# zichunhao/lgn-autoencoder

Measured on AMD Instinct MI355X. Metric: jets/sec fwd+bwd, 30-particle maxdim=2 bs=512, higher is better.
Workload: dtype f64

## Files before the change

### include/lgn_amd.h

```cpp
#ifndef LGN_AMD_H
#define LGN_AMD_H

#include <stddef.h>
#include <stdint.h>

#ifdef __cplusplus
extern "C" {
#endif

#define LGN_AMD_ABI_VERSION 19

int lgn_abi_version(void);
const char* lgn_last_error(void);

int lgn_level_fwd_f64(int B, int N, int C, int CO, int decoder,
                      const double* s_in, const double* v_in, const double* p, const uint8_t* mask,
                      const double* ra, const double* rb, const double* rc,
                      const double* w0, const double* b0, const double* w1, const double* b1,
                      const double* wm0, const double* wm1,
                      double* ag0, double* ag1, double* s_out, double* v_out, void* stream);

int lgn_level_bwd_partial_rows(int B, int N, int decoder, int* rows_mix, int* rows_rad);
int lgn_level_rad_partial_len(int C, int decoder);
int lgn_level_jet_split(int B, int N);
// ... 51 lines not shown
  int n_rows, n_out, n_w;
  int n_terms, n_u, n_x;
  int n_units, static_kind;
  const int *row_ptr, *t_type, *t_a, *t_b;
  const double* t_coef;
  const int *out_dim, *out_nblk, *out_row0, *out_q0, *out_w0;
  const int *u_ptr, *u_row;
  const double* u_coef;
  const int *x_ptr, *x_row, *x_other;
  const double* x_coef;
  int h_out_w0[8];
} lgn_local_tables;

int lgn_local_fwd_f64(int nodes, int C, int CO, int Q, int Qout, const lgn_local_tables* t, const double* X, const double* U,
                      const double* wcat, double* out, void* stream);
int lgn_local_partial_rows(int nodes);
int lgn_local_bwd_f64(int nodes, int C, int CO, int Q, int Qout, const lgn_local_tables* t, const double* X, const double* U,
                      const double* wcat, const double* g_out, double* gU, double* gX, double* part, void* stream);

long long lgn_local_static_packed_doubles(int kind, int C, int CO);
int lgn_local_bwd_static_f64(int kind, int nodes, int C, int CO, const double* XT, const double* UT, const double* wcat,
                             const int* w0, double* wpacked, const double* goT, double* gUT, double* gXT, double* part,
                             double* gpacked, double* g_wcat, void* stream);
int lgn_local_fwd_static_f64(int kind, int nodes, int C, int CO, const double* XT, const double* UT, const double* wcat,
                             const int* w0, double* wpacked, double* outT, double* s_copy, int q_s, void* stream);

typedef struct lgn_net_desc {
  int B, N;
  int n_levels;
  int enc_channels[5];
  int dec_channels[5];
  int tau_s, tau_v;
  int mlp_hidden_mul;
  int mlp_nlin;
  int tau_v_in;
  const lgn_local_tables* enc_tables[4];
  const lgn_local_tables* dec_tables[4];
  int enc_Q[5], enc_qs[5], enc_qv[5];
  int dec_Q[5], dec_qs[5], dec_qv[5];
  int flags;
  int activation;
  int n_in_scalars;
  int latent_pool;
  int dec_N;
  int get_real;
  double jet_loss_scale;
} lgn_net_desc;
#define LGN_REAL_SUM 0
#define LGN_REAL_REAL 1
#define LGN_REAL_IMAG 2
#define LGN_REAL_MEAN 3
#define LGN_REAL_NORM 4
#define LGN_LOSS_CHAMFER 0
#define LGN_LOSS_MSE 1
#define LGN_LOSS_HUNGARIAN 2
typedef struct lgn_loss_desc {
  int kind;
  int abs_coord;
  int polar_coord;
  double scale;
} lgn_loss_desc;
#define LGN_POOL_MIN 0
#define LGN_POOL_MAX 1
#define LGN_POOL_MEAN 2
#define LGN_POOL_MIX 3
#define LGN_POOL(n, avg, o0, o1, o2, o3) ((n) | ((avg) << 3) | ((o0) << 4) | ((o1) << 6) | ((o2) << 8) | ((o3) << 10))
#define LGN_NET_NO_STATIC 1
#define LGN_NET_DEC_PAIRWISE 2
#define LGN_NET_LEVEL_V2 4
#define LGN_NET_MLP_V1 8
#define LGN_NET_MOMENTS_V1 16
#define LGN_NET_BWD_ORDERED 64
#define LGN_NET_DEC_UNFUSED 256
#define LGN_NET_MOMENTS_SPLIT 512
#define LGN_NET_MLP_BWD1 1024
#define LGN_NET_MLP_FULLTILE 2048
#define LGN_NET_LIVE_SCALARS 4096
#define LGN_NET_SPLIT_TAIL 128

#define LGN_LDS_LIMIT (160 * 1024)
long long lgn_encoder_end_lds_bytes(int N, int C0, int K, int CL, int Ts, int Tv, int pool);
long long lgn_decoder_end_lds_bytes(int N, int C0, int Tin, int CL);
long long lgn_junction_lds_bytes(int N, int CL, int Ts, int Tv, int pool, int C0);

int lgn_step_param_slots(const lgn_net_desc* d, int decoder);
long long lgn_step_workspace_doubles(const lgn_net_desc* d);
int lgn_step_fwd_bwd_f64(const lgn_net_desc* d, const double* params, double* grads, long long n_params,
                         const int64_t* enc_off, const int64_t* dec_off, const double* p4, const double* target,
                         const uint8_t* mask, const double* in_scalars, double* workspace, long long workspace_doubles,
                         double* recon, double* loss_part, const lgn_loss_desc* loss, int* assignment ,
                         int* status , void* stream);
#define LGN_FINALIZE_SCRATCH 2048
int lgn_step_finalize_f64(double* params, double* grads, long long n_params, const double* loss_part, int n_loss,
                          double l1_lambda, double* adam_m, double* adam_v, long long* step_dev,
                          double lr, double beta1, double beta2, double eps, int do_adam, double* loss_out, void* stream);
int lgn_step_train_f64(const lgn_net_desc* d, double* params, double* grads, long long n_params, const int64_t* enc_off,
                       const int64_t* dec_off, const double* p4, const double* target, const uint8_t* mask, const double* in_scalars,
                       double* workspace, long long workspace_doubles, double* recon, double* loss_part, int n_loss, double l1_lambda,
                       double* adam_m, double* adam_v, long long* step_dev, double lr, double beta1, double beta2, double eps,
                       int do_adam, double* loss_out, const lgn_loss_desc* loss, int* assignment ,
                       int* status , void* stream);

#define LGN_OPT_ADAM 0
#define LGN_OPT_RMSPROP 1
typedef struct {
  int kind;
  double l1_lambda, l2_lambda, lr, eps;
  double beta1, beta2;
  double alpha, momentum;
} lgn_optim_desc;
#define LGN_FINALIZE_OPT_SCRATCH 4096
int lgn_step_finalize_opt_f64(double* params, double* grads, long long n_params, const double* loss_part, int n_loss,
                              const lgn_optim_desc* opt, double* state_m, double* state_v, long long* step_dev, int do_step,
                              double* loss_out, void* stream);
int lgn_step_train_opt_f64(const lgn_net_desc* d, double* params, double* grads, long long n_params, const int64_t* enc_off,
                           const int64_t* dec_off, const double* p4, const double* target, const uint8_t* mask,
                           const double* in_scalars, double* workspace, long long workspace_doubles, double* recon,
                           double* loss_part, int n_loss, const lgn_optim_desc* opt, double* state_m, double* state_v,
                           long long* step_dev, int do_step, double* loss_out, const lgn_loss_desc* loss,
                           int* assignment , int* status , void* stream);

long long lgn_eval_workspace_doubles(const lgn_net_desc* d);
int lgn_step_eval_f64(const lgn_net_desc* d, const double* params, const int64_t* enc_off, const int64_t* dec_off,
                      const double* p4_scaled, const double* p4_target, const uint8_t* mask, const double* in_scalars,
                      double* workspace, long long workspace_doubles, double* recon_real, double* lat_s ,
                      double* lat_v , double* loss_part, double* loss_out, const lgn_loss_desc* loss,
                      int* assignment , int* status , void* stream);

long long lgn_net_workspace_doubles(const lgn_net_desc* d, int decoder, int which);
int lgn_encoder_fwd_f64(const lgn_net_desc* d, const double* params, const int64_t* off, const double* p4, const uint8_t* mask,
                        const double* in_scalars, double* act, long long act_doubles, double* lat_s, double* lat_v, void* stream);
int lgn_encoder_bwd_f64(const lgn_net_desc* d, const double* params, double* grads, long long n_params, const int64_t* off,
                        const double* p4, const uint8_t* mask, const double* in_scalars, const double* act, long long act_doubles,
                        const double* g_lat_s, const double* g_lat_v, double* scratch, long long scratch_doubles, void* stream);
int lgn_decoder_fwd_f64(const lgn_net_desc* d, const double* params, const int64_t* off, const double* lat_v, double* act,
                        long long act_doubles, double* recon, void* stream);
int lgn_decoder_bwd_f64(const lgn_net_desc* d, const double* params, double* grads, long long n_params, const int64_t* off,
                        const double* lat_v, const double* act, long long act_doubles, const double* g_recon, double* g_lat_v,
                        double* scratch, long long scratch_doubles, void* stream);

int lgn_chamfer_f64(int B, int N, int M, const double* x, const double* y, int jet_features, double* loss_part, double* gx, double* gy,
                    void* stream);

#define LGN_ANOMALY_NMAX 192
#define LGN_ANOMALY_NSCORES 21
#define LGN_ANOMALY_ALL 0x1FFFFF
#define LGN_ANOMALY_HUNGARIAN 0x403E0
#define LGN_ANOMALY_NO_HUNGARIAN (LGN_ANOMALY_ALL & ~LGN_ANOMALY_HUNGARIAN)
int lgn_anomaly_scores_f64(const double* recons, const double* target, const double* recons_n, const double* target_n, int B, int N,
                           int score_mask, double* scores, int* col4row , int* status, void* stream);

#define LGN_ROC_TILE 2048
#define LGN_ROC_MAX_COLS 65535
#define LGN_ROC_NONFINITE 1
#define LGN_ROC_SINGLE_CLASS 2
#define LGN_ROC_BAD_LABEL 4
#define LGN_ROC_NAN 8
long long lgn_roc_workspace_bytes(long long M, int K);
int lgn_roc_auc_f64(const double* scores, long long M, int ld, int K, const double* labels, double* fpr, double* tpr,
                    double* thresholds, int* length, double* auc, int* flipped, int* status, void* workspace,
                    long long workspace_bytes, void* stream);

#define LGN_EMD_NMAX 191
#define LGN_EMD_INVALID 1
#define LGN_EMD_EMPTY 2
#define LGN_EMD_ITER 4
// ... 112 lines not shown
```

### lgn-autoencoder_amd/csrc/level.hpp

```cpp
#pragma once
#include "common.hpp"

namespace lgn {

constexpr int LVL_DEC_PAIRWISE = 2;
constexpr int LVL_LEVEL_V2 = 4;
constexpr int LVL_MLP_V1 = 8;
constexpr int LVL_MOMENTS_V1 = 16;
constexpr int LVL_MLP_BWD1 = 1024;
constexpr int LVL_MLP_FULLTILE = 2048;
constexpr int LVL_MOMENTS_SPLIT = 512;
constexpr int LVL_LIVE_SCALARS = 4096;
constexpr int LVL_DEC_STORE_AG = 16384;
constexpr int LVL_BWD_ORDERED = 64;
int level_flags_from_env();

template <typename T>
struct LevelArgs {
  int B, N, C, CO;
  const T* s_in;
  const T* v_in;
  const T* p;
  const uint8_t* mask;
  const T *ra, *rb, *rc, *w0, *b0, *w1, *b1;
  const T *wm0, *wm1;
  T* ag0;
  T* ag1;
  T* s_out;
  T* v_out;
  const T* in_w0 = nullptr;
  const T* in_w1 = nullptr;
  T* in_s = nullptr;
  T* in_v = nullptr;
  T* z1 = nullptr;
  size_t z1n = 0;
  T* z2 = nullptr;
  size_t z2n = 0;
  const T* loss_wo1 = nullptr;
  const T* loss_target = nullptr;
  T loss_scale = T(1);
  int loss_real = 0;
  T loss_jscale = T(0);
  T* loss_recon = nullptr;
  T* loss_part = nullptr;
  T* loss_gv = nullptr;
  T* loss_wpart = nullptr;
  int flags = 0;
  int dead_scalars = 0;
  T* sep_sums = nullptr;
};
constexpr int sep_sums_doubles(int C) { return 20 * C + 8; }

template <typename T>
struct LevelBwdArgs {
  int B, N, C, CO;
  const T *s_in, *v_in, *p;
  const uint8_t* mask;
  const T *ra, *rb, *rc, *w0, *b0, *w1, *b1;
  const T *wm0, *wm1;
  const T *ag0, *ag1;
  const T* g_s_out;
  const T* g_v_out;
  T* g_ag;
  T* g_s_in;
  T* g_v_in;
  T* g_p;
  T* part_mix;
  T* part_rad;
  T* part_in0 = nullptr;
  int flags = 0;
  int dead_scalars = 0;
  const T* sep_sums = nullptr;
};

__host__ __device__ constexpr int node_stride(int C) { return 10 * C + 4; }

__host__ __device__ constexpr int rad_partial_size(int C, bool dec) {
  return dec ? 2 * C : (2 * 4 * C * NB + 8 * C);
}

inline int level_jet_split(int B, int N) {
  const int groups = (N + 3) / 4;
  int s = 1;
  while (s * 2 <= groups && B * s * 2 <= 512) s *= 2;
  return s;
}

}
```

### lgn-autoencoder_amd/csrc/level_fwd2.hip

```cpp
#include "level_dev.hpp"
#include "net_dev.hpp"
#include "ops.hpp"
#include "wave_sum.hpp"

namespace lgn {

LGN_STAMP_DECL
LGN_STAMP_READER(lgn_debug_stamps_fwd2)

template <int C, bool DEC>
struct Fwd2 {
  static constexpr int NG = (C + 3) / 4;
  static constexpr int NS = node_stride(C);
  static constexpr int PS = DEC ? 8 : 4;
  static constexpr int AGS = 20 * C;
  static constexpr int A3 = 0, A4 = 2 * C, A1 = 4 * C, A2 = 12 * C;
};

template <int C, bool DEC, bool SEP, bool TRAIN, bool NOS>
__global__ __launch_bounds__(2 * BLOCK) void level_fwd2_kernel(LevelArgs<double> a, int chunk) {
  using F = Fwd2<C, DEC>;
  constexpr int NG = F::NG;
  const int N = a.N, B = a.B, CO = a.CO;
  const int b = blockIdx.x, tid = threadIdx.x, lane = tid & 63, wave = tid >> 6;
  const int nthr = blockDim.x, nw = nthr >> 6;

  extern __shared__ __align__(16) unsigned char smem_raw[];
  double* nd = reinterpret_cast<double*>(smem_raw);
  double* pj = nd + ((N * F::NS + 1) & ~1);
  double* wm = pj + N * F::PS;
  double* agl = wm + 4 * CO * 5 * C;
  double* sums = agl + chunk * F::AGS;
  uint8_t* mk = reinterpret_cast<uint8_t*>(sums + 20 * C);

  STAMP(0);
  if (!DEC && a.in_w0) {
    {
      const size_t wg = (size_t)blockIdx.y * gridDim.x + blockIdx.x, stride = (size_t)gridDim.x * gridDim.y * nthr;
      for (size_t e = wg * nthr + tid; e < a.z1n; e += stride) a.z1[e] = 0.0;
      for (size_t e = wg * nthr + tid; e < a.z2n; e += stride) a.z2[e] = 0.0;
    }
    const double* p0 = a.p + (size_t)b * N * 4;
    const size_t plane_s = (size_t)B * N * C;
    const int nw2 = 2 * CO * 5 * C;
    for (int e = tid; e < N * 4; e += nthr) pj[e] = p0[e];
    for (int e = tid; e < N; e += nthr) mk[e] = a.mask[(size_t)b * N + e];
    for (int e = tid; e < nw2; e += nthr) {
      wm[e] = a.wm0[e];
      wm[nw2 + e] = a.wm1[e];
    }
    for (int e = tid; e < N * C; e += nthr) {
      const int j = e / C, c = e - j * C;
      const double* p = p0 + j * 4;
      const double pe = p[0], px = p[1], py = p[2], pz = p[3];
      const double mass = sqrt(fabs(minkowski_sq_unfused(pe, px, py, pz)));
      constexpr double H = 0.70710678118654752440084436210484903928;
      const cx<double> q[4] = {{pe, 0.0}, {px * H, -py * H}, {pz, 0.0}, {-px * H, -py * H}};
      const double w0r = a.in_w0[c], w0i = a.in_w0[C + c];
      const cx<double> w1 = {a.in_w1[c], a.in_w1[C + c]};
      double* d = nd + j * F::NS + c * 10;
      d[0] = w0r * mass;
      d[1] = w0i * mass;
#pragma unroll
      for (int m = 0; m < 4; ++m) {
        const cx<double> r = cmul(w1, q[m]);
        d[2 + m] = r.r;
        d[6 + m] = r.i;
      }
      if (blockIdx.y == 0) {
        const size_t ge = (size_t)b * N * C + e;
        a.in_s[ge] = d[0];
        a.in_s[plane_s + ge] = d[1];
#pragma unroll
        for (int m = 0; m < 4; ++m) {
          a.in_v[ge * 4 + m] = d[2 + m];
          a.in_v[plane_s * 4 + ge * 4 + m] = d[6 + m];
        }
      }
    }
  } else {
    JetRegs<double> jr;
    load_jet_issue<double, C, DEC>(a.s_in, a.v_in, a.p, a.mask, B, N, b, jr);
    const int nw2 = 2 * CO * 5 * C, ew = tid < nw2 ? tid : 0;
    const double w0v = a.wm0[ew], w1v = a.wm1[ew];
    load_jet_commit<double, C, DEC>(a.s_in, a.v_in, a.p, a.mask, B, N, b, jr, nd, pj, mk);
    if (tid < nw2) {
      wm[tid] = w0v;
      wm[nw2 + tid] = w1v;
    }
    for (int e = tid + nthr; e < nw2; e += nthr) {
      wm[e] = a.wm0[e];
      wm[nw2 + e] = a.wm1[e];
    }
  }

  const int pr = lane & 15, cg = lane >> 4;
  const int ti = pr >> 2, tj = pr & 3;
  double ak[5], bk[5], ck2[5];
  double wf[NG][5];
  double bias[NG][4];
  if (!DEC) {
#pragma unroll
    for (int s = 0; s < 5; ++s) {
      const int k = 4 * s + cg;
      ak[s] = a.ra[k];
      bk[s] = a.rb[k];
      const double c = a.rc[k];
      ck2[s] = c * c;
    }
#pragma unroll
    for (int g = 0; g < NG; ++g) {
      const int rr = lane & 15, q = rr >> 2, ch = 4 * g + (rr & 3);
      const double* w = (q >> 1) ? a.w1 : a.w0;
#pragma unroll
      for (int s = 0; s < 5; ++s) wf[g][s] = ch < C ? w[(2 * ch + (q & 1)) * NB + 4 * s + cg] : 0.0;
    }
  }
#pragma unroll
  for (int g = 0; g < NG; ++g) {
    const int ch = 4 * g + cg;
#pragma unroll
    for (int q = 0; q < 4; ++q) {
      const double* bb = (q >> 1) ? a.b1 : a.b0;
      bias[g][q] = ch < C ? (DEC ? bb[ch] : bb[2 * ch + (q & 1)]) : 0.0;
    }
  }
  __syncthreads();
  STAMP(1);

  if constexpr (DEC && SEP) {
    if (tid < 64) {
      const int k = tid & 7, part = tid >> 3;
      double mean = 0.0;
      for (int n = part; n < N; n += 8) mean += pj[n * 8 + k];
      mean += shfl_xor(mean, 8);
      mean += shfl_xor(mean, 16);
      mean += shfl_xor(mean, 32);
      if (part == 0) {
        const double mu = mean / N;
        sums[k] = mu;
        if constexpr (TRAIN) {
          if (a.sep_sums) a.sep_sums[(size_t)b * sep_sums_doubles(C) + 20 * C + k] = mu;
        }
      }
    }
    __syncthreads();
    for (int e = tid; e < N * 8; e += nthr) pj[e] -= sums[e & 7];
    __syncthreads();
#define LGN_PUT(k, val)                                           \
  do {                                                            \
    if ((k) < 12) a0[(k) < 12 ? (k) : 0] += (val);                \
    else a1[(k) >= 12 ? (k) - 12 : 0] += (val);                   \
  } while (0)
    for (int c = wave; c < C; c += nw) {
      double a0[12], a1[8];
#pragma unroll
      for (int k = 0; k < 12; ++k) a0[k] = 0.0;
#pragma unroll
      for (int k = 0; k < 8; ++k) a1[k] = 0.0;
      for (int n = lane; n < N; n += 64) {
        const double* ni = nd + n * F::NS + c * 10;
// ... 252 lines not shown
        A4[g].r = quad_sum(A4[g].r);        A4[g].i = quad_sum(A4[g].i);
      }
#pragma unroll
      for (int m = 0; m < 4; ++m) {
        A1[g][m].r = quad_sum(A1[g][m].r);  A1[g][m].i = quad_sum(A1[g][m].i);
        A2[g][m].r = quad_sum(A2[g][m].r);  A2[g][m].i = quad_sum(A2[g][m].i);
      }
    }
    if (tj == 0) {
      double* st = agl + (slab + i0 + ti - c0) * F::AGS;
#pragma unroll
      for (int g = 0; g < NG; ++g) {
        const int ch = 4 * g + cg;
        if (ch < C) {
          if constexpr (!NOS) {
            st[F::A3 + 2 * ch] = A3[g].r;  st[F::A3 + 2 * ch + 1] = A3[g].i;
            st[F::A4 + 2 * ch] = A4[g].r;  st[F::A4 + 2 * ch + 1] = A4[g].i;
          }
#pragma unroll
          for (int m = 0; m < 4; ++m) {
            st[F::A1 + (ch * 4 + m) * 2] = A1[g][m].r;  st[F::A1 + (ch * 4 + m) * 2 + 1] = A1[g][m].i;
            st[F::A2 + (ch * 4 + m) * 2] = A2[g][m].r;  st[F::A2 + (ch * 4 + m) * 2 + 1] = A2[g][m].i;
          }
        }
      }
    }
    STAMP(4 + ((rg >> 2) & 3) * 4);
  };
  if (rs > 1) {
    const int rg = (c0 >> 2) + wave / rs;
    if (rg * 4 < c1) row_group(rg, 4 * (rpart * ntl / rs), min(N, 4 * ((rpart + 1) * ntl / rs)), rpart * 4 * ngr);
  } else {
    for (int rg = (c0 >> 2) + wave; rg * 4 < c1; rg += nw) row_group(rg, 0, N, 0);
  }
  if (rs > 1) {
    __syncthreads();
    const int tot = 4 * ngr * F::AGS;
    for (int e = tid; e < tot; e += nthr) {
      if (NOS && e % F::AGS < F::A1) continue;
      double v = agl[e];
      for (int pp = 1; pp < rs; ++pp) v += agl[pp * tot + e];
      agl[e] = v;
    }
  }
  }
  __syncthreads();
  STAMP(20);

  if (TRAIN && !(DEC && SEP && a.sep_sums)) {
    const size_t pl0 = (size_t)B * N * 2 * C;
    if constexpr (!NOS) {
      for (int e = tid; e < (c1 - c0) * 2 * C; e += nthr) {
        const int n = e / (2 * C), r = e - n * 2 * C, blk = r / C, ch = r - blk * C;
        const double* st = agl + n * F::AGS + (blk ? F::A4 : F::A3) + 2 * ch;
        const size_t ge = ((size_t)b * N + c0) * 2 * C + e;
        a.ag0[ge] = st[0];
        a.ag0[pl0 + ge] = st[1];
      }
    }
    for (int e = tid; e < (c1 - c0) * 2 * C * 4; e += nthr) {
      const int n = e / (8 * C), r = e - n * 8 * C, blk = r / (4 * C), cm = r - blk * 4 * C;
      const double* st = agl + n * F::AGS + (blk ? F::A2 : F::A1) + 2 * cm;
      const size_t ge = ((size_t)b * N + c0) * 8 * C + e;
      a.ag1[ge] = st[0];
      a.ag1[pl0 * 4 + ge] = st[1];
    }
  }
  STAMP(21);

  catmix(c0, c1);
  STAMP(22);
  if (c1 < rhi) __syncthreads();
  }
  STAMP(40);
  if constexpr (DEC) {
    if (a.loss_wo1) {
      __syncthreads();
      dec_output_loss_body<TRAIN>(B, N, CO, a.v_out, a.loss_wo1, a.loss_target, a.loss_scale, a.loss_real, a.loss_jscale,
                                  a.loss_recon, a.loss_part, a.loss_gv, a.loss_wpart, smem_raw);
    }
  }
}

template <int C, bool DEC, bool SEP, bool TRAIN, bool NOS>
static int launch_level_fwd2(const LevelArgs<double>& a, hipStream_t stream) {
  using F = Fwd2<C, DEC>;
  const size_t fixed = sizeof(double) * (((size_t)a.N * F::NS + 1 & ~size_t(1)) + (size_t)a.N * F::PS + 4 * a.CO * 5 * C + 20 * C) + a.N + 16;
  const bool wide = a.B <= 320 && a.N >= 64;
  const size_t row = sizeof(double) * F::AGS, budget1 = 160 * 1024, budget2 = wide ? budget1 : 78 * 1024;
  const int full = (a.N + 15) & ~15;
  int chunk = full;
  if (fixed + full * row > budget2) {
    const size_t room = fixed + 16 * row <= budget2 ? budget2 - fixed : (fixed < budget1 ? budget1 - fixed : 0);
    chunk = (int)(room / row) & ~15;
    if (chunk > full) chunk = full;
    if (chunk < 16) chunk = 16;
  }
  size_t smem = fixed + chunk * row;
  if (a.loss_wo1) {
    LGN_CHECK_ARG(DEC && SEP && a.N <= 40 && !wide && a.loss_target && a.loss_recon && a.loss_part && (!TRAIN || (a.loss_gv && a.loss_wpart)),
                  "level_fwd: the loss rides on the separable decoder forward of jets of <= 40 particles only");
    if (smem < dec_out_loss_bytes(a.N, a.CO)) smem = dec_out_loss_bytes(a.N, a.CO);
  }
  LGN_CHECK_ARG(!a.sep_sums || (DEC && SEP && TRAIN && a.N <= 40),
                "level_fwd: only the separable decoder forward of a training step (N <= 40) leaves jet sums instead of the aggregate");
  LGN_CHECK_ARG(smem <= 160 * 1024, "level_fwd: N=%d C=%d needs %zu B of LDS (> 160 KiB)", a.N, a.C, smem);
  auto kern = level_fwd2_kernel<C, DEC, SEP, TRAIN, NOS>;
  if (smem > 64 * 1024) {
    hipError_t e = hipFuncSetAttribute(reinterpret_cast<const void*>(kern), hipFuncAttributeMaxDynamicSharedMemorySize, (int)smem);
    if (e != hipSuccess) { set_error("hipFuncSetAttribute: %s", hipGetErrorString(e)); return (int)e; }
  }
  const int nthreads = wide ? 2 * BLOCK : BLOCK;
  const int split = (SEP || a.N > 40) ? 1 : level_jet_split(a.B, a.N);
  hipLaunchKernelGGL(kern, dim3(a.B, split), dim3(nthreads), smem, stream, a, chunk);
  LGN_CHECK_LAUNCH();
  return 0;
}

bool level_fwd_carries_loss(int N, int flags) { return N <= 40 && !(flags & LVL_DEC_PAIRWISE); }

template <bool TRAIN, bool NOS>
static int level_fwd_run(const LevelArgs<double>& a, int decoder, hipStream_t stream) {
  LGN_CHECK_ARG(a.B > 0 && a.N > 0, "level_fwd: empty batch (B=%d N=%d)", a.B, a.N);
  LGN_CHECK_ARG(!a.in_w0 || (!decoder && a.in_w1 && a.in_s && a.in_v), "level_fwd: the input stage rides on encoder levels only");
  LGN_CHECK_ARG(a.CO >= 1 && a.CO <= 8, "level_fwd: C_out=%d unsupported (1..8)", a.CO);
  const bool pairwise = (a.flags & LVL_DEC_PAIRWISE) != 0;
#define LGN_CASE(CC)                                                                                         \
  case CC:                                                                                                   \
    if (!decoder) return launch_level_fwd2<CC, false, false, TRAIN, NOS>(a, stream);                         \
    return pairwise ? launch_level_fwd2<CC, true, false, TRAIN, NOS>(a, stream) : launch_level_fwd2<CC, true, true, TRAIN, NOS>(a, stream);
  switch (a.C) {
#ifdef LGN_DEV_ONLY_C4
    LGN_CASE(4)
#else
    LGN_CASE(1) LGN_CASE(2) LGN_CASE(3) LGN_CASE(4) LGN_CASE(5) LGN_CASE(6) LGN_CASE(7) LGN_CASE(8)
#endif
    default:
      set_error("level_fwd: C_in=%d unsupported (1..8)", a.C);
      return -1;
  }
#undef LGN_CASE
}

template <>
int level_fwd_dispatch<double>(const LevelArgs<double>& a, int decoder, hipStream_t stream) {
  return a.dead_scalars ? level_fwd_run<true, true>(a, decoder, stream) : level_fwd_run<true, false>(a, decoder, stream);
}

int level_fwd_eval(const LevelArgs<double>& a, int decoder, hipStream_t stream) {
  return a.dead_scalars ? level_fwd_run<false, true>(a, decoder, stream) : level_fwd_run<false, false>(a, decoder, stream);
}

}
```

### lgn-autoencoder_amd/csrc/net_dev.hpp

```cpp
#pragma once
#include "common.hpp"

namespace lgn {

constexpr double NET_RSQRT2 = 0.70710678118654752440084436210484903928;

__device__ __forceinline__ void cart_from_canon_bwd(const cx<double> (&g)[4], cx<double> (&gc)[4]) {
  gc[0] = g[0];
  gc[1] = {(g[1].r + g[2].i) * NET_RSQRT2, (g[1].i - g[2].r) * NET_RSQRT2};
  gc[2] = g[3];
  gc[3] = {(-g[1].r + g[2].i) * NET_RSQRT2, (-g[1].i - g[2].r) * NET_RSQRT2};
}

__device__ __forceinline__ double block_sum(double v, double* red) {
  v = group_sum<64>(v);
  if ((threadIdx.x & 63) == 0) red[threadIdx.x >> 6] = v;
  __syncthreads();
  double s = (red[0] + red[1]) + (red[2] + red[3]);
  __syncthreads();
  return s;
}
template <int U>
struct StageRegs {
  double r[U];
  __device__ __forceinline__ void issue(const double* __restrict__ src, int total) {
#pragma unroll
    for (int u = 0; u < U; ++u) r[u] = total > 0 ? src[min((int)threadIdx.x + u * BLOCK, total - 1)] : 0.0;
  }
  template <class Put>
  __device__ __forceinline__ void commit(const double* __restrict__ src, int total, Put put) const {
#pragma unroll
    for (int u = 0; u < U; ++u)
      if ((int)threadIdx.x + u * BLOCK < total) put((int)threadIdx.x + u * BLOCK, r[u]);
    for (int e = threadIdx.x + U * BLOCK; e < total; e += BLOCK) put(e, src[e]);
  }
};
__device__ __forceinline__ cx<double> cart_from_canon_m(const double* c, int m) {
  if (m == 0) return {c[0], c[4]};
  if (m == 3) return {c[2], c[6]};
  if (m == 1) return {(c[1] - c[3]) * NET_RSQRT2, (c[5] - c[7]) * NET_RSQRT2};
  return {-(c[5] + c[7]) * NET_RSQRT2, (c[1] + c[3]) * NET_RSQRT2};
}

__device__ __forceinline__ void jet_sums(const double* x, int N, const double* y, int M, double* js) {
  const int tid = threadIdx.x;
  if (tid < 8) {
    const int m = tid & 3;
    double s = 0.0;
    if (tid < 4) for (int i = 0; i < N; ++i) s += x[i * 4 + m];
    else for (int j = 0; j < M; ++j) s += y[j * 4 + m];
    js[tid] = s;
  }
}

enum : int { REAL_SUM = 0, REAL_RE = 1, REAL_IM = 2, REAL_MEAN = 3, REAL_NORM = 4 };
constexpr double GET_REAL_NORM_EPS = 1e-16;

__host__ __device__ inline size_t dec_out_loss_bytes(int N, int C) {
  return sizeof(double) * ((size_t)N * 22 + (size_t)N * C * 10 + 2 * (size_t)C + 8) + sizeof(int) * 2 * (size_t)N;
}
template <bool GRAD = true>
__device__ __forceinline__ void dec_output_loss_body(int B, int N, int C, const double* __restrict__ v,
                                                     const double* __restrict__ wo1, const double* __restrict__ target,
                                                     double loss_scale, int method, double jscale, double* recon,
                                                     double* loss_part, double* g_v, double* part, unsigned char* smem_raw) {
  double* x = reinterpret_cast<double*>(smem_raw);
  double* tg = x + N * 4;
  double* rmin = tg + N * 4;
  double* cmin = rmin + N;
  double* gx = cmin + N;
  double* ycl = gx + N * 4;
  double* vl = ycl + N * 8;
  double* tmp = vl + N * C * 8;
  double* wol = tmp + N * C * 2;
  int* rarg = reinterpret_cast<int*>(wol + 2 * C);
  int* carg = rarg + N;
  double* js = reinterpret_cast<double*>(carg + N);
  __shared__ double red[4];
  const int b = blockIdx.x;
  const size_t plp = (size_t)B * N * 4, pl = (size_t)B * N * C, j4 = (size_t)b * N * 4, jc = (size_t)b * N * C;
  {
    StageRegs<4> vr, vi;
    StageRegs<1> tr, wr;
    vr.issue(v + jc * 4, N * C * 4); vi.issue(v + (pl + jc) * 4, N * C * 4); tr.issue(target + j4, N * 4); wr.issue(wo1, 2 * C);
// ... 124 lines not shown
  double *x = s.x, *tg = s.tg, *ycl = s.ycl, *vl = s.vl, *wol = s.wol;
  const int b = blockIdx.x;
  const size_t plp = (size_t)B * N * 4, pl = (size_t)B * N * C, j4 = (size_t)b * N * 4, jc = (size_t)b * N * C;
  {
    StageRegs<4> vr, vi;
    StageRegs<1> tr, wr;
    vr.issue(v + jc * 4, N * C * 4); vi.issue(v + (pl + jc) * 4, N * C * 4); tr.issue(target + j4, N * 4); wr.issue(wo1, 2 * C);
    vr.commit(v + jc * 4, N * C * 4, [&](int e, double q) { vl[(e >> 2) * 8 + (e & 3)] = q; });
    vi.commit(v + (pl + jc) * 4, N * C * 4, [&](int e, double q) { vl[(e >> 2) * 8 + 4 + (e & 3)] = q; });
    tr.commit(target + j4, N * 4, [&](int e, double q) { tg[e] = q; });
    wr.commit(wo1, 2 * C, [&](int e, double q) { wol[e] = q; });
  }
  __syncthreads();
  for (int e = threadIdx.x; e < N * 4; e += BLOCK) {
    const int n = e >> 2, m = e & 3;
    cx<double> yc = {0, 0};
#pragma unroll 4
    for (int c = 0; c < C; ++c)
      cfma(yc, cx<double>{wol[c], wol[C + c]}, cx<double>{vl[(n * C + c) * 8 + m], vl[(n * C + c) * 8 + 4 + m]});
    ycl[n * 8 + m] = yc.r;
    ycl[n * 8 + 4 + m] = yc.i;
  }
  __syncthreads();
  for (int e = threadIdx.x; e < N * 4; e += BLOCK) {
    const cx<double> pc = cart_from_canon_m(ycl + (e >> 2) * 8, e & 3);
    if (GRAD) {
      recon[j4 + e] = pc.r;
      recon[plp + j4 + e] = pc.i;
    }
    double xe;
    if (method == REAL_SUM) xe = pc.r + pc.i;
    else if (method == REAL_RE) xe = pc.r;
    else if (method == REAL_IM) xe = pc.i;
    else if (method == REAL_MEAN) xe = (pc.r + pc.i) / 2;
    else xe = sqrt(pc.r * pc.r + pc.i * pc.i + GET_REAL_NORM_EPS);
    x[e] = xe;
    if (!GRAD) recon[j4 + e] = xe;
  }
  __syncthreads();
}
__device__ __forceinline__ void dec_out_backward(int B, int N, int C, int method, double* g_v, double* part, const DecOutLds& s) {
  double *x = s.x, *gx = s.gx, *ycl = s.ycl, *vl = s.vl, *tmp = s.tmp, *wol = s.wol;
  const int b = blockIdx.x;
  const size_t pl = (size_t)B * N * C, jc = (size_t)b * N * C;
  for (int e = threadIdx.x; e < N * C; e += BLOCK) {
    const int n = e / C, c = e - n * C;
    cx<double> g[4], gc[4], d = {0, 0};
#pragma unroll
    for (int m = 0; m < 4; ++m) {
      const double q = gx[n * 4 + m];
      if (method == REAL_SUM) g[m] = {q, q};
      else if (method == REAL_RE) g[m] = {q, 0.0};
      else if (method == REAL_IM) g[m] = {0.0, q};
      else if (method == REAL_MEAN) g[m] = {q / 2, q / 2};
      else {
        const cx<double> pc = cart_from_canon_m(ycl + n * 8, m);
        const double r = q / x[n * 4 + m];
        g[m] = {r * pc.r, r * pc.i};
      }
    }
    cart_from_canon_bwd(g, gc);
    const cx<double> w = {wol[c], wol[C + c]};
    const size_t base = jc + e;
#pragma unroll
    for (int m = 0; m < 4; ++m) {
      cx<double> r = cmulc(gc[m], w);
      g_v[base * 4 + m] = r.r;
      g_v[pl * 4 + base * 4 + m] = r.i;
      cfmac(d, gc[m], cx<double>{vl[e * 8 + m], vl[e * 8 + 4 + m]});
    }
    tmp[e * 2] = d.r;
    tmp[e * 2 + 1] = d.i;
  }
  __syncthreads();
  if ((int)threadIdx.x < 2 * C) {
    const int k = threadIdx.x / C, c = threadIdx.x - k * C;
    double acc = 0.0;
#pragma unroll 6
    for (int n = 0; n < N; ++n) acc += tmp[(n * C + c) * 2 + k];
    part[(size_t)b * 2 * C + k * C + c] = acc;
  }
}

}
```

### lgn-autoencoder_amd/csrc/net_kernels.hip

```cpp
#include "net.hpp"
#include "net_dev.hpp"
#include "tail_dev.hpp"

namespace lgn {

LGN_STAMP_DECL
LGN_STAMP_READER(lgn_debug_stamps_net)

namespace {
constexpr double H = 0.70710678118654752440084436210484903928;

__device__ __forceinline__ double minkowski_sq_ref(const double* p) {
  return minkowski_sq_unfused(p[0], p[1], p[2], p[3]);
}
__device__ __forceinline__ void canon_real(const double* p, cx<double> (&q)[4]) {
  q[0] = {p[0], 0.0};
  q[1] = {p[1] * H, -p[2] * H};
  q[2] = {p[3], 0.0};
  q[3] = {-p[1] * H, -p[2] * H};
}
__device__ __forceinline__ void canon_cplx(const cx<double> (&p)[4], cx<double> (&c)[4]) {
  c[0] = p[0];
  c[1] = {(p[1].r + p[2].i) * H, (p[1].i - p[2].r) * H};
  c[2] = p[3];
  c[3] = {(-p[1].r + p[2].i) * H, (-p[1].i - p[2].r) * H};
}
__device__ __forceinline__ void canon_cplx_bwd(const cx<double> (&g)[4], cx<double> (&gp)[4]) {
  gp[0] = g[0];
  gp[1] = {(g[1].r - g[3].r) * H, (g[1].i - g[3].i) * H};
  gp[2] = {-(g[1].i + g[3].i) * H, (g[1].r + g[3].r) * H};
  gp[3] = g[2];
}
__device__ __forceinline__ void cart_from_canon(const cx<double> (&c)[4], cx<double> (&p)[4]) {
  p[0] = c[0];
  p[1] = {(c[1].r - c[3].r) * H, (c[1].i - c[3].i) * H};
  p[2] = {-(c[1].i + c[3].i) * H, (c[1].r + c[3].r) * H};
  p[3] = c[2];
}
}

__global__ void enc_input_fwd_kernel(int B, int N, int C, int K, const double* __restrict__ p4, const double* __restrict__ xs,
                                     const double* __restrict__ w0, const double* __restrict__ w1, double* s, double* v, double* z1,
                                     size_t n1, double* z2, size_t n2) {
  const size_t total = (size_t)B * N * C, pl = total;
  for (size_t e = (size_t)blockIdx.x * blockDim.x + threadIdx.x; e < n1; e += (size_t)gridDim.x * blockDim.x) z1[e] = 0.0;
  for (size_t e = (size_t)blockIdx.x * blockDim.x + threadIdx.x; e < n2; e += (size_t)gridDim.x * blockDim.x) z2[e] = 0.0;
  for (size_t e = (size_t)blockIdx.x * blockDim.x + threadIdx.x; e < total; e += (size_t)gridDim.x * blockDim.x) {
    const int c = e % C;
    const size_t node = e / C;
    const double* p = p4 + node * 4;
    const double mass = sqrt(fabs(minkowski_sq_ref(p)));
    cx<double> q[4];
    canon_real(p, q);
    double sr = w0[c * K] * mass, si = w0[(C + c) * K] * mass;
    for (int k = 1; k < K; ++k) {
      const double x = xs[node * (K - 1) + (k - 1)];
      sr = __builtin_fma(w0[c * K + k], x, sr);
      si = __builtin_fma(w0[(C + c) * K + k], x, si);
    }
    s[e] = sr;
    s[pl + e] = si;
    const cx<double> w = {w1[c], w1[C + c]};
#pragma unroll
    for (int m = 0; m < 4; ++m) {
      cx<double> r = cmul(w, q[m]);
      v[e * 4 + m] = r.r;
      v[pl * 4 + e * 4 + m] = r.i;
    }
  }
}

__global__ __launch_bounds__(BLOCK) void enc_input_bwd_kernel(int B, int N, int C, int K, const double* __restrict__ p4,
                                                             const double* __restrict__ xs, const double* __restrict__ g_s,
                                                             const double* __restrict__ g_v, double* part) {
  extern __shared__ __align__(16) unsigned char smem_raw[];
  double* tmp = reinterpret_cast<double*>(smem_raw);
  const int T = 2 * K + 2;
  const int b = blockIdx.x;
  const size_t pl = (size_t)B * N * C;
  for (int i = threadIdx.x; i < N * C; i += BLOCK) {
    const int n = i / C;
    const double* p = p4 + ((size_t)b * N + n) * 4;
    const double mass = sqrt(fabs(minkowski_sq_ref(p)));
    cx<double> q[4];
    canon_real(p, q);
    const size_t e = (size_t)b * N * C + i;
    cx<double> d1 = {0, 0};
#pragma unroll
    for (int m = 0; m < 4; ++m) cfmac(d1, cx<double>{g_v[e * 4 + m], g_v[pl * 4 + e * 4 + m]}, q[m]);
    const double gr = g_s[e], gi = g_s[pl + e];
    tmp[i * T + 0] = gr * mass;
    tmp[i * T + K] = gi * mass;
    for (int k = 1; k < K; ++k) {
      const double x = xs[((size_t)b * N + n) * (K - 1) + (k - 1)];
      tmp[i * T + k] = gr * x;
      tmp[i * T + K + k] = gi * x;
    }
    tmp[i * T + 2 * K] = d1.r;
    tmp[i * T + 2 * K + 1] = d1.i;
  }
  __syncthreads();
  for (int o = threadIdx.x; o < T * C; o += BLOCK) {
    int c, t;
    if (o < 2 * C * K) {
      const int z = o / (C * K), r = o - z * C * K;
      c = r / K;
      t = z * K + (r - c * K);
    } else {
      const int r = o - 2 * C * K, z = r / C;
      c = r - z * C;
      t = 2 * K + z;
    }
    double acc = 0.0;
    for (int n = 0; n < N; ++n) acc += tmp[(n * C + c) * T + t];
    part[(size_t)b * T * C + o] = acc;
  }
}

__device__ __forceinline__ cx<double> canon_cplx_m(const double* p, int m) {
  if (m == 0) return {p[0], p[4]};
  if (m == 2) return {p[3], p[7]};
  const double sg = m == 1 ? 1.0 : -1.0;
  return {(sg * p[1] + p[6]) * H, (sg * p[5] - p[2]) * H};
}
__device__ __forceinline__ cx<double> canon_cplx_bwd_m(const double* g, int m) {
  if (m == 0) return {g[0], g[4]};
  if (m == 3) return {g[2], g[6]};
  if (m == 1) return {(g[1] - g[3]) * H, (g[5] - g[7]) * H};
  return {-(g[5] + g[7]) * H, (g[1] + g[3]) * H};
}

__host__ __device__ inline size_t lat_y_doubles(int N, int Ts, int Tv, int pool = 0) {
  return (size_t)(pool_is_mix(pool) ? 1 : N) * (2 * Ts + 8 * Tv);
}
__host__ __device__ inline size_t lat_fwd_doubles(int N, int C, int Ts, int Tv, int pool = 0) {
  return lat_y_doubles(N, Ts, Tv, pool) + (size_t)N * C * 10 + 2 * (size_t)(Ts + Tv) * pool_mix_in(pool, N, C);
}
struct LatentStage {
  StageRegs<2> sr, si;
  StageRegs<4> vr, vi;
  StageRegs<1> w0, w1;
  const double *s0, *s1, *v0, *v1, *wl0, *wl1;
  int N, C, Ts, Tv, K, NY, NS;
  __device__ __forceinline__ void issue(int B, int N_, int C_, int Ts_, int Tv_, const double* __restrict__ s, const double* __restrict__ v,
                                        const double* __restrict__ wl0_, const double* __restrict__ wl1_, int pool = 0) {
    N = N_; C = C_; Ts = Ts_; Tv = Tv_; wl0 = wl0_; wl1 = wl1_; K = pool_mix_in(pool, N_, C_); NY = (int)lat_y_doubles(N_, Ts_, Tv_, pool);
    const size_t pl = (size_t)B * N * C, j0 = (size_t)blockIdx.x * N * C;
    NS = s ? N * C : 0;
    s0 = s ? s + j0 : nullptr; s1 = s ? s + pl + j0 : nullptr; v0 = v + j0 * 4; v1 = v + (pl + j0) * 4;
    vr.issue(v0, N * C * 4); vi.issue(v1, N * C * 4);
    sr.issue(s0, NS); si.issue(s1, NS);
    w0.issue(wl0, 2 * Ts * K); w1.issue(wl1, 2 * Tv * K);
  }
  __device__ __forceinline__ void commit(double* lds, bool zero_y) const {
    double* sv = lds + NY;
    double* w0l = sv + N * C * 10;
    double* w1l = w0l + 2 * Ts * K;
    if (zero_y)
      for (int e = threadIdx.x; e < NY; e += BLOCK) lds[e] = 0.0;
    vr.commit(v0, N * C * 4, [&](int e, double x) { sv[(e >> 2) * 10 + 2 + (e & 3)] = x; });
    vi.commit(v1, N * C * 4, [&](int e, double x) { sv[(e >> 2) * 10 + 6 + (e & 3)] = x; });
    if (NS) {
      sr.commit(s0, NS, [&](int e, double x) { sv[e * 10] = x; });
      si.commit(s1, NS, [&](int e, double x) { sv[e * 10 + 1] = x; });
    } else {
      for (int e = threadIdx.x; e < N * C; e += BLOCK) sv[e * 10] = sv[e * 10 + 1] = 0.0;
    }
    w0.commit(wl0, 2 * Ts * K, [&](int e, double x) { w0l[e] = x; });
    w1.commit(wl1, 2 * Tv * K, [&](int e, double x) { w1l[e] = x; });
  }
};
template <bool TO_LDS>
__device__ __forceinline__ void enc_latent_fwd_body(int B, int N, int C, int Ts, int Tv, int pool, double* lat_s, double* lat_v, int* idx,
                                                    double* lds, double* lat_l) {
  const int b = blockIdx.x, TT = Ts + Tv;
  const int P = pool_blocks(pool), PN = pool_n(pool);
  bool need_mean = false;
  for (int i = 0; i < PN; ++i) need_mean |= pool_op(pool, i) == LGN_POOL_MEAN;
  const int YS = 2 * Ts + 8 * Tv;
  double* y = lds;
  const double* sv = y + N * YS;
  const double* w0l = sv + N * C * 10;
  const double* w1l = w0l + 2 * Ts * C;
  STAMP(1);
  for (int e = threadIdx.x; e < N * Tv; e += BLOCK) {
    const int n = e / Tv, tv = e - n * Tv;
    const double* x = sv + n * C * 10;
    cx<double> acc[4] = {{0, 0}, {0, 0}, {0, 0}, {0, 0}}, pc[4];
#pragma unroll 4
    for (int c = 0; c < C; ++c) {
      const cx<double> w = {w1l[tv * C + c], w1l[Tv * C + tv * C + c]};
#pragma unroll
      for (int m = 0; m < 4; ++m) cfma(acc[m], w, cx<double>{x[c * 10 + 2 + m], x[c * 10 + 6 + m]});
    }
    cart_from_canon(acc, pc);
    double* o = y + n * YS + 2 * Ts + 8 * tv;
#pragma unroll
    for (int m = 0; m < 4; ++m) { o[m] = pc[m].r; o[4 + m] = pc[m].i; }
  }
  for (int e = threadIdx.x; e < N * Ts; e += BLOCK) {
    const int n = e / Ts, t = e - n * Ts;
    const double* x = sv + n * C * 10;
    cx<double> acc = {0, 0};
#pragma unroll 4
    for (int c = 0; c < C; ++c) cfma(acc, cx<double>{w0l[t * C + c], w0l[Ts * C + t * C + c]}, cx<double>{x[c * 10], x[c * 10 + 1]});
    y[n * YS + 2 * t] = acc.r;
    y[n * YS + 2 * t + 1] = acc.i;
  }
  __syncthreads();
  STAMP(2);
  const int l8 = threadIdx.x & 7;
  constexpr int NONE = 0x7fffffff;
  for (int it = threadIdx.x >> 3; it < 2 * TT; it += BLOCK / 8) {
    const int z = it / TT, t = it - z * TT;
    int imin = NONE, imax = NONE;
    double smin = 0, smax = 0;
#pragma unroll 4
    for (int n = l8; n < N; n += 8) {
      double lo, hi;
      if (t < Ts) {
        const double val = y[n * YS + 2 * t + z];
        lo = val;
        hi = val * val;
      } else {
        const double* o = y + n * YS + 2 * Ts + 8 * (t - Ts) + 4 * z;
        lo = hi = o[0] * o[0] - ((o[1] * o[1] + o[2] * o[2]) + o[3] * o[3]);
      }
      if (imin == NONE || lo < smin) { smin = lo; imin = n; }
      if (imax == NONE || hi > smax) { smax = hi; imax = n; }
    }
#pragma unroll
    for (int off = 4; off; off >>= 1) {
      const double om = __shfl_xor(smin, off, 8), oM = __shfl_xor(smax, off, 8);
      const int oi = __shfl_xor(imin, off, 8), oI = __shfl_xor(imax, off, 8);
      if (oi != NONE && (imin == NONE || om < smin || (om == smin && oi < imin))) { smin = om; imin = oi; }
      if (oI != NONE && (imax == NONE || oM > smax || (oM == smax && oI < imax))) { smax = oM; imax = oI; }
    }
    imin = __shfl(imin, 0, 8);
    imax = __shfl(imax, 0, 8);
    if (l8 < 2) idx[(((size_t)b * 2 + z) * TT + t) * 2 + l8] = l8 ? imax : imin;
    const int nc = t < Ts ? 1 : 4, y0 = t < Ts ? 2 * t + z : 2 * Ts + 8 * (t - Ts) + 4 * z;
    double mean[4] = {0, 0, 0, 0};
    if (need_mean) {
      for (int n = l8; n < N; n += 8)
#pragma unroll
        for (int m = 0; m < 4; ++m)
          if (m < nc) mean[m] += y[n * YS + y0 + m];
#pragma unroll
      for (int off = 4; off; off >>= 1)
#pragma unroll
        for (int m = 0; m < 4; ++m) mean[m] += __shfl_xor(mean[m], off, 8);
#pragma unroll
      for (int m = 0; m < 4; ++m) mean[m] /= (double)N;
    }
    for (int k = l8; k < P * nc; k += 8) {
      const int pb = k / nc, m = k - pb * nc;
      auto pick = [&](int op) -> double {
        if (op == LGN_POOL_MIN) return y[imin * YS + y0 + m];
        if (op == LGN_POOL_MAX) return y[imax * YS + y0 + m];
        return m == 0 ? mean[0] : (m == 1 ? mean[1] : (m == 2 ? mean[2] : mean[3]));
      };
      double val;
      if (pool_avg(pool)) {
        val = pick(pool_op(pool, 0));
        for (int i = 1; i < PN; ++i) val += pick(pool_op(pool, i));
        val /= (double)PN;
      } else {
        val = pick(pool_op(pool, pb));
      }
      if (t < Ts) {
        lat_s[((size_t)z * B + b) * P * Ts + pb * Ts + t] = val;
      } else {
        const int tv = t - Ts;
        lat_v[(((size_t)z * B + b) * P * Tv + pb * Tv + tv) * 4 + m] = val;
        if constexpr (TO_LDS) lat_l[(pb * Tv + tv) * 8 + 4 * z + m] = val;
      }
    }
  }
}
template <bool TO_LDS>
__device__ __forceinline__ void enc_latent_mix_fwd_body(int B, int N, int C, int Ts, int Tv, double* lat_s, double* lat_v, double* lds,
                                                        double* lat_l) {
  const int b = blockIdx.x, TT = Ts + Tv, K = N * C;
  const double* sv = lds + (2 * Ts + 8 * Tv);
  const double* w0l = sv + K * 10;
  const double* w1l = w0l + 2 * Ts * K;
  const int l8 = threadIdx.x & 7;
  for (int t = threadIdx.x >> 3; t < TT; t += BLOCK / 8) {
    if (t < Ts) {
      cx<double> acc = {0, 0};
      for (int k = l8; k < K; k += 8) cfma(acc, cx<double>{w0l[t * K + k], w0l[Ts * K + t * K + k]}, cx<double>{sv[k * 10], sv[k * 10 + 1]});
#pragma unroll
      for (int off = 4; off; off >>= 1) { acc.r += __shfl_xor(acc.r, off, 8); acc.i += __shfl_xor(acc.i, off, 8); }
      if (l8 < 2) lat_s[((size_t)l8 * B + b) * Ts + t] = l8 ? acc.i : acc.r;
    } else {
      const int tv = t - Ts;
      cx<double> acc[4] = {{0, 0}, {0, 0}, {0, 0}, {0, 0}}, pc[4];
      for (int k = l8; k < K; k += 8) {
        const cx<double> w = {w1l[tv * K + k], w1l[Tv * K + tv * K + k]};
#pragma unroll
        for (int m = 0; m < 4; ++m) cfma(acc[m], w, cx<double>{sv[k * 10 + 2 + m], sv[k * 10 + 6 + m]});
      }
#pragma unroll
      for (int off = 4; off; off >>= 1)
#pragma unroll
        for (int m = 0; m < 4; ++m) { acc[m].r += __shfl_xor(acc[m].r, off, 8); acc[m].i += __shfl_xor(acc[m].i, off, 8); }
      cart_from_canon(acc, pc);
      const int z = l8 >> 2, m = l8 & 3;
      const cx<double> pm = m == 0 ? pc[0] : (m == 1 ? pc[1] : (m == 2 ? pc[2] : pc[3]));
      const double val = z ? pm.i : pm.r;
      lat_v[(((size_t)z * B + b) * Tv + tv) * 4 + m] = val;
      if constexpr (TO_LDS) lat_l[tv * 8 + 4 * z + m] = val;
    }
  }
}
__global__ __launch_bounds__(BLOCK) void enc_latent_fwd_kernel(int B, int N, int C, int Ts, int Tv, int pool,
                                                              const double* __restrict__ s, const double* __restrict__ v,
                                                              const double* __restrict__ wl0, const double* __restrict__ wl1,
                                                              double* lat_s, double* lat_v, int* idx) {
  extern __shared__ __align__(16) unsigned char smem_raw[];
  double* lds = reinterpret_cast<double*>(smem_raw);
  LatentStage st;
  st.issue(B, N, C, Ts, Tv, s, v, wl0, wl1, pool);
  st.commit(lds, false);
  __syncthreads();
  if (pool_is_mix(pool)) enc_latent_mix_fwd_body<false>(B, N, C, Ts, Tv, lat_s, lat_v, lds, nullptr);
  else enc_latent_fwd_body<false>(B, N, C, Ts, Tv, pool, lat_s, lat_v, idx, lds, nullptr);
}

constexpr int LAT_PARTS = 6;
__host__ __device__ inline size_t lat_bwd_doubles(int N, int C, int Ts, int Tv, int pool = 0) {
  return lat_fwd_doubles(N, C, Ts, Tv, pool) + (pool_is_mix(pool) ? 0 : (size_t)LAT_PARTS * (Ts + Tv) * C * 2);
}
struct LatentBwdPrefetch {
  int n[2];
  double gs[4];
  bool valid;
  __device__ __forceinline__ void issue(int B, int Ts, int Tv, int pool, const int* __restrict__ idx, const double* __restrict__ g_lat_s) {
    const int TT = Ts + Tv, e = threadIdx.x, b = blockIdx.x, P = pool_blocks(pool);
    valid = 2 * TT <= BLOCK && !pool_is_mix(pool);
    if (valid && e < 2 * TT) {
      const int z = e / TT, t = e - z * TT;
#pragma unroll
      for (int kind = 0; kind < 2; ++kind) n[kind] = idx[(((size_t)b * 2 + z) * TT + t) * 2 + kind];
#pragma unroll
      for (int pb = 0; pb < 4; ++pb) gs[pb] = (t < Ts && pb < P) ? g_lat_s[((size_t)z * B + b) * P * Ts + pb * Ts + t] : 0.0;
    }
  }
};
template <bool FROM_LDS>
__device__ __forceinline__ void enc_latent_bwd_body(int B, int N, int C, int Ts, int Tv, int pool, const double* __restrict__ g_lat_s,
                                                    const double* __restrict__ g_lat_v, const double* g_lat_l,
                                                    const int* __restrict__ idx, double* g_s, double* g_v, double* part, double* lds,
                                                    const LatentBwdPrefetch& pre) {
  const int b = blockIdx.x, TT = Ts + Tv;
  const int YS = 2 * Ts + 8 * Tv;
  double* gy = lds;
  const double* sv = gy + N * YS;
  const double* w0l = sv + N * C * 10;
  const double* w1l = w0l + 2 * Ts * C;
  double* red = const_cast<double*>(w1l) + 2 * Tv * C;
  const size_t pl = (size_t)B * N * C;
// ... 105 lines not shown
    } else {
      row[2 * Ts * C + (t - Ts) * C + c] = ar;
      row[2 * Ts * C + Tv * C + (t - Ts) * C + c] = ai;
    }
  }
}
template <bool FROM_LDS>
__device__ __forceinline__ void enc_latent_mix_bwd_body(int B, int N, int C, int Ts, int Tv, const double* __restrict__ g_lat_s,
                                                        const double* __restrict__ g_lat_v, const double* g_lat_l, double* g_s, double* g_v,
                                                        double* part, double* lds) {
  const int b = blockIdx.x, TT = Ts + Tv, K = N * C;
  double* gy = lds;
  const double* sv = lds + (2 * Ts + 8 * Tv);
  const double* w0l = sv + K * 10;
  const double* w1l = w0l + 2 * Ts * K;
  const size_t pl = (size_t)B * K;
  for (int t = threadIdx.x; t < TT; t += BLOCK) {
    if (t < Ts) {
      gy[2 * t] = g_lat_s ? g_lat_s[((size_t)0 * B + b) * Ts + t] : 0.0;
      gy[2 * t + 1] = g_lat_s ? g_lat_s[((size_t)1 * B + b) * Ts + t] : 0.0;
    } else {
      const int tv = t - Ts;
      cx<double> g[4], gc[4];
      for (int m = 0; m < 4; ++m) {
        if constexpr (FROM_LDS) g[m] = {g_lat_l[tv * 8 + m], g_lat_l[tv * 8 + 4 + m]};
        else g[m] = {g_lat_v[(((size_t)0 * B + b) * Tv + tv) * 4 + m], g_lat_v[(((size_t)1 * B + b) * Tv + tv) * 4 + m]};
      }
      cart_from_canon_bwd(g, gc);
      double* o = gy + 2 * Ts + 8 * tv;
      for (int m = 0; m < 4; ++m) { o[m] = gc[m].r; o[4 + m] = gc[m].i; }
    }
  }
  __syncthreads();
  for (int k = threadIdx.x; k < K; k += BLOCK) {
    cx<double> as = {0, 0}, av[4] = {{0, 0}, {0, 0}, {0, 0}, {0, 0}};
    for (int t = 0; t < Ts; ++t) cfmac(as, cx<double>{gy[2 * t], gy[2 * t + 1]}, cx<double>{w0l[t * K + k], w0l[Ts * K + t * K + k]});
    for (int t = 0; t < Tv; ++t) {
      const cx<double> w = {w1l[t * K + k], w1l[Tv * K + t * K + k]};
      const double* o = gy + 2 * Ts + 8 * t;
#pragma unroll
      for (int m = 0; m < 4; ++m) cfmac(av[m], cx<double>{o[m], o[4 + m]}, w);
    }
    const size_t base = (size_t)b * K + k;
    g_s[base] = as.r;
    g_s[pl + base] = as.i;
#pragma unroll
    for (int m = 0; m < 4; ++m) { g_v[base * 4 + m] = av[m].r; g_v[pl * 4 + base * 4 + m] = av[m].i; }
  }
  double* row = part + (size_t)b * 2 * TT * K;
  for (int e = threadIdx.x; e < TT * K; e += BLOCK) {
    const int t = e / K, k = e - t * K;
    cx<double> acc = {0, 0};
    if (t < Ts) {
      cfmac(acc, cx<double>{gy[2 * t], gy[2 * t + 1]}, cx<double>{sv[k * 10], sv[k * 10 + 1]});
      row[t * K + k] = acc.r;
      row[Ts * K + t * K + k] = acc.i;
    } else {
      const int tv = t - Ts;
      const double* o = gy + 2 * Ts + 8 * tv;
#pragma unroll
      for (int m = 0; m < 4; ++m) cfmac(acc, cx<double>{o[m], o[4 + m]}, cx<double>{sv[k * 10 + 2 + m], sv[k * 10 + 6 + m]});
      row[2 * Ts * K + tv * K + k] = acc.r;
      row[2 * Ts * K + Tv * K + tv * K + k] = acc.i;
    }
  }
}
__global__ __launch_bounds__(BLOCK) void enc_latent_bwd_kernel(int B, int N, int C, int Ts, int Tv, int pool,
                                                              const double* __restrict__ s, const double* __restrict__ v,
                                                              const double* __restrict__ wl0, const double* __restrict__ wl1,
                                                              const double* __restrict__ g_lat_s, const double* __restrict__ g_lat_v,
                                                              const int* __restrict__ idx, double* g_s, double* g_v, double* part) {
  extern __shared__ __align__(16) unsigned char smem_raw[];
  double* lds = reinterpret_cast<double*>(smem_raw);
  LatentStage st;
  LatentBwdPrefetch pre;
  st.issue(B, N, C, Ts, Tv, s, v, wl0, wl1, pool);
  pre.issue(B, Ts, Tv, pool, idx, g_lat_s);
  st.commit(lds, true);
  __syncthreads();
  if (pool_is_mix(pool)) enc_latent_mix_bwd_body<false>(B, N, C, Ts, Tv, g_lat_s, g_lat_v, nullptr, g_s, g_v, part, lds);
  else enc_latent_bwd_body<false>(B, N, C, Ts, Tv, pool, g_lat_s, g_lat_v, nullptr, idx, g_s, g_v, part, lds, pre);
}

__host__ __device__ inline size_t dec_in_fwd_doubles(int N, int C, int Tin) {
  return 2 * (size_t)N * Tin + (size_t)Tin * 8 + (size_t)N * 8 + 4 * (size_t)C;
}
struct DecInFwdStage {
  StageRegs<4> wg;
  StageRegs<1> a0, a1, lr, li;
  const double *wg1, *w0, *w1, *l0, *l1;
  int N, C, Tin;
  bool with_lat;
  __device__ __forceinline__ void issue(int B, int N_, int C_, int Tin_, const double* __restrict__ lat_v, const double* __restrict__ wg1_,
                                        const double* __restrict__ w0_, const double* __restrict__ w1_, bool with_lat_) {
    N = N_; C = C_; Tin = Tin_; wg1 = wg1_; w0 = w0_; w1 = w1_; with_lat = with_lat_;
    wg.issue(wg1, 2 * N * Tin);
    a0.issue(w0, 2 * C); a1.issue(w1, 2 * C);
    if (with_lat) {
      l0 = lat_v + (size_t)blockIdx.x * Tin * 4; l1 = lat_v + ((size_t)B + blockIdx.x) * Tin * 4;
      lr.issue(l0, Tin * 4); li.issue(l1, Tin * 4);
    }
  }
  __device__ __forceinline__ void commit(double* lds) const {
    double* wgl = lds;
    double* latl = wgl + 2 * N * Tin;
    double* w01 = latl + Tin * 8 + N * 8;
    wg.commit(wg1, 2 * N * Tin, [&](int e, double x) { wgl[e] = x; });
    a0.commit(w0, 2 * C, [&](int e, double x) { w01[e] = x; });
    a1.commit(w1, 2 * C, [&](int e, double x) { w01[2 * C + e] = x; });
    if (with_lat) {
      lr.commit(l0, Tin * 4, [&](int e, double x) { latl[(e >> 2) * 8 + (e & 3)] = x; });
      li.commit(l1, Tin * 4, [&](int e, double x) { latl[(e >> 2) * 8 + 4 + (e & 3)] = x; });
    }
  }
};
__device__ __forceinline__ void dec_input_fwd_body(int B, int N, int C, int Tin, double* pdec, double* s0, double* v0, double* lds) {
  const double* wgl = lds;
  const double* latl = wgl + 2 * N * Tin;
  double* cartl = const_cast<double*>(latl) + Tin * 8;
  const double* w01 = cartl + N * 8;
  const int b = blockIdx.x;
  const size_t plp = (size_t)B * N * 4, pl = (size_t)B * N * C;
  STAMP(3);
  for (int e = threadIdx.x; e < N * 4; e += BLOCK) {
    const int n = e >> 2, m = e & 3;
    cx<double> acc = {0, 0};
#pragma unroll 8
    for (int t = 0; t < Tin; ++t)
      cfma(acc, cx<double>{wgl[n * Tin + t], wgl[N * Tin + n * Tin + t]}, cx<double>{latl[t * 8 + m], latl[t * 8 + 4 + m]});
    cartl[n * 8 + m] = acc.r;
    cartl[n * 8 + 4 + m] = acc.i;
  }
  __syncthreads();
  STAMP(4);
  for (int e = threadIdx.x; e < N * 4; e += BLOCK) {
    const cx<double> pc = canon_cplx_m(cartl + (e >> 2) * 8, e & 3);
    pdec[(size_t)b * N * 4 + e] = pc.r;
    pdec[plp + (size_t)b * N * 4 + e] = pc.i;
  }
  for (int e = threadIdx.x; e < N * C; e += BLOCK) {
    const int c = e % C;
    s0[(size_t)b * N * C + e] = w01[c] - w01[C + c];
    s0[pl + (size_t)b * N * C + e] = w01[C + c] + w01[c];
  }
  for (int e = threadIdx.x; e < N * C * 4; e += BLOCK) {
    const int i = e >> 2, m = e & 3, n = i / C, c = i - n * C;
    const cx<double> r = cmul(cx<double>{w01[2 * C + c], w01[3 * C + c]}, canon_cplx_m(cartl + n * 8, m));
    v0[(size_t)b * N * C * 4 + e] = r.r;
    v0[pl * 4 + (size_t)b * N * C * 4 + e] = r.i;
  }
}
__global__ __launch_bounds__(BLOCK) void dec_input_fwd_kernel(int B, int N, int C, int Tin, const double* __restrict__ lat_v,
                                                             const double* __restrict__ wg1, const double* __restrict__ w0,
                                                             const double* __restrict__ w1, double* pdec, double* s0, double* v0) {
  extern __shared__ __align__(16) unsigned char smem_raw[];
  double* lds = reinterpret_cast<double*>(smem_raw);
  DecInFwdStage st;
  st.issue(B, N, C, Tin, lat_v, wg1, w0, w1, true);
  st.commit(lds);
  __syncthreads();
  dec_input_fwd_body(B, N, C, Tin, pdec, s0, v0, lds);
}

__host__ __device__ inline size_t dec_in_bwd_doubles(int N, int C, int Tin) {
  return (size_t)N * 16 + 2 * (size_t)N * Tin + (size_t)Tin * 8 + (size_t)N * 16 + (size_t)N * C * 10 + 2 * (size_t)C;
}
struct DecInBwdStage {
  StageRegs<4> gvr, gvi, wg;
  StageRegs<1> gpr, gpi, pdr, pdi, gsr, gsi, lr, li, a1;
  const double *gv0, *gv1, *wg1, *gp0, *gp1, *pd0, *pd1, *gs0, *gs1, *l0, *l1, *w1;
  int N, C, Tin;
  __device__ __forceinline__ void issue(int B, int N_, int C_, int Tin_, const double* __restrict__ lat_v, const double* __restrict__ wg1_,
                                        const double* __restrict__ w1_, const double* __restrict__ pdec, const double* __restrict__ g_p,
                                        const double* __restrict__ g_s0, const double* __restrict__ g_v0) {
    N = N_; C = C_; Tin = Tin_; wg1 = wg1_; w1 = w1_;
    const int b = blockIdx.x;
    const size_t plp = (size_t)B * N * 4, pl = (size_t)B * N * C, j4 = (size_t)b * N * 4, jc = (size_t)b * N * C;
    gv0 = g_v0 + jc * 4; gv1 = g_v0 + (pl + jc) * 4; gp0 = g_p + j4; gp1 = g_p + plp + j4; pd0 = pdec + j4; pd1 = pdec + plp + j4;
    gs0 = g_s0 + jc; gs1 = g_s0 + pl + jc; l0 = lat_v + (size_t)b * Tin * 4; l1 = lat_v + ((size_t)B + b) * Tin * 4;
    gvr.issue(gv0, N * C * 4); gvi.issue(gv1, N * C * 4); wg.issue(wg1, 2 * N * Tin);
    gpr.issue(gp0, N * 4); gpi.issue(gp1, N * 4); pdr.issue(pd0, N * 4); pdi.issue(pd1, N * 4);
    gsr.issue(gs0, N * C); gsi.issue(gs1, N * C); lr.issue(l0, Tin * 4); li.issue(l1, Tin * 4); a1.issue(w1, 2 * C);
  }
  __device__ __forceinline__ void commit(double* lds) const {
    double* wgl = lds + N * 16;
    double* latl = wgl + 2 * N * Tin;
    double* gp_l = latl + Tin * 8;
    double* pd_l = gp_l + N * 8;
    double* gs_l = pd_l + N * 8;
    double* gv_l = gs_l + N * C * 2;
    double* w1l = gv_l + N * C * 8;
    gvr.commit(gv0, N * C * 4, [&](int e, double x) { gv_l[(e >> 2) * 8 + (e & 3)] = x; });
    gvi.commit(gv1, N * C * 4, [&](int e, double x) { gv_l[(e >> 2) * 8 + 4 + (e & 3)] = x; });
    wg.commit(wg1, 2 * N * Tin, [&](int e, double x) { wgl[e] = x; });
    gpr.commit(gp0, N * 4, [&](int e, double x) { gp_l[(e >> 2) * 8 + (e & 3)] = x; });
    gpi.commit(gp1, N * 4, [&](int e, double x) { gp_l[(e >> 2) * 8 + 4 + (e & 3)] = x; });
    pdr.commit(pd0, N * 4, [&](int e, double x) { pd_l[(e >> 2) * 8 + (e & 3)] = x; });
    pdi.commit(pd1, N * 4, [&](int e, double x) { pd_l[(e >> 2) * 8 + 4 + (e & 3)] = x; });
    gsr.commit(gs0, N * C, [&](int e, double x) { gs_l[e * 2] = x; });
    gsi.commit(gs1, N * C, [&](int e, double x) { gs_l[e * 2 + 1] = x; });
    lr.commit(l0, Tin * 4, [&](int e, double x) { latl[(e >> 2) * 8 + (e & 3)] = x; });
    li.commit(l1, Tin * 4, [&](int e, double x) { latl[(e >> 2) * 8 + 4 + (e & 3)] = x; });
    a1.commit(w1, 2 * C, [&](int e, double x) { w1l[e] = x; });
  }
};
template <bool TO_LDS>
__device__ __forceinline__ void dec_input_bwd_body(int B, int N, int C, int Tin, double* g_lat_v, double* part, double* lds, double* g_lat_l) {
  double* gcan = lds;
  double* gcart = gcan + N * 8;
  const double* wgl = gcart + N * 8;
  const double* latl = wgl + 2 * N * Tin;
  const double* gp_l = latl + Tin * 8;
  const double* pd_l = gp_l + N * 8;
  const double* gs_l = pd_l + N * 8;
  double* gv_l = const_cast<double*>(gs_l) + N * C * 2;
  const double* w1l = gv_l + N * C * 8;
  const int b = blockIdx.x;
  double* row = part + (size_t)b * (4 * C + 2 * N * Tin);
  STAMP(11);
  for (int e = threadIdx.x; e < N * 4; e += BLOCK) {
    const int n = e >> 2, m = e & 3;
    cx<double> g = {gp_l[n * 8 + m], gp_l[n * 8 + 4 + m]};
#pragma unroll 4
    for (int c = 0; c < C; ++c)
      cfmac(g, cx<double>{gv_l[(n * C + c) * 8 + m], gv_l[(n * C + c) * 8 + 4 + m]}, cx<double>{w1l[c], w1l[C + c]});
    gcan[n * 8 + m] = g.r;
    gcan[n * 8 + 4 + m] = g.i;
  }
  __syncthreads();
  for (int i = threadIdx.x; i < N * C; i += BLOCK) {
    const int n = i / C;
    cx<double> d0 = {0, 0}, d1 = {0, 0};
    cfmac(d0, cx<double>{gs_l[i * 2], gs_l[i * 2 + 1]}, cx<double>{1.0, 1.0});
#pragma unroll
// ... 586 lines not shown
```

### lgn-autoencoder_amd/csrc/ops.hpp

```cpp
#pragma once
#include <cstdlib>
#include <vector>
#include "level.hpp"

namespace lgn {

template <typename T> int level_fwd_dispatch(const LevelArgs<T>&, int decoder, hipStream_t);
int level_fwd_eval(const LevelArgs<double>&, int decoder, hipStream_t);
template <typename T> int level_bwd_dispatch(const LevelBwdArgs<T>&, int decoder, hipStream_t);
template <typename T> int reduce_partials(const T* part, int rows, int n, T* out, int accumulate, hipStream_t);
template <typename T> int reduce_partials_strided(const T* part, int rows, int stride, int col0, int n, T* out, hipStream_t);
constexpr int RED_MAX_SEG = 64;
template <typename T> struct RedSeg { const T* part; int rows, stride, col0, n; T* out; };
template <typename T> struct RedJob {
  int nseg;
  RedSeg<T> seg[RED_MAX_SEG];
  int tile0[RED_MAX_SEG + 1];
  void add(const T* part, int rows, int stride, int col0, int n, T* out) { seg[nseg++] = RedSeg<T>{part, rows, stride, col0, n, out}; }
};
template <typename T> int reduce_segments(RedJob<T>& job, hipStream_t);
template <typename T>
int rad_finalize(const T* tot, int C, const T* ra, const T* rb, const T* rc, const T* w0, const T* w1, T* g_a, T* g_b, T* g_c,
                 T* g_w0, T* g_b0, T* g_w1, T* g_b1, hipStream_t);
struct RadFinJob {
  int n;
  struct Item { const double* tot; int C; const double *ra, *rb, *rc, *w0, *w1; double *g_a, *g_b, *g_c, *g_w0, *g_b0, *g_w1, *g_b1; } it[4];
};
int rad_finalize_batch(const RadFinJob& job, hipStream_t);
struct StepTailArgs {
  double *w, *g;
  long n;
  double *m, *v;
  long* step_dev;
  double lambda, lr, beta1, beta2, eps;
  int do_adam;
  const double* loss_part;
  int nB;
  double* loss_out;
  int reduce_only;
  unsigned long long* counters;
  int opt_form = 0;
  int kind = 0;
  double l2 = 0.0, alpha = 0.0, mu = 0.0;
};
int step_tail(const std::vector<RedSeg<double>>& segs, const RadFinJob& fin, const StepTailArgs& ta, hipStream_t st);
void level_bwd_partial_rows(int B, int N, int decoder, int flags, int* rows_mix, int* rows_rad);
bool level_bwd_carries_input(int N, int flags);
bool level_dec_rebuilds(int N, int flags);
bool level_fwd_carries_loss(int N, int flags);

constexpr int MLP_MAX_LIN = 8;
template <typename T>
struct MlpArgs {
  int M;
  int C;
  int H;
  int nlin;
  const T* w[MLP_MAX_LIN];
  const T* b[MLP_MAX_LIN];
  const T* s_in;
  T* s_out;
  const T* g_out;
  T* g_in;
  T* part;
  int psize;
  int ld = 1;
  int tbQ = 0;
  T* h_saved = nullptr;
  int h_rows = 0;
  int act = 0;
  int flags = 0;
};
inline int mlp_saved_rows(int M) { return (M + 63) & ~63; }
inline size_t mlp_saved_doubles(int M, int H, int nlin) {
  return H <= 48 && nlin >= 4 && nlin <= 7 ? (size_t)(nlin - 1) * mlp_saved_rows(M) * ((H + 15) & ~15) : 0;
}
constexpr int MLP_SAVE_MAX_ROWS = 8128;
inline size_t mlp_save_max_rows() {
  static const long v = [] { const char* e = getenv("LGN_AMD_MLP_SAVE_ROWS"); return e ? atol(e) : (long)MLP_SAVE_MAX_ROWS; }();
  return (size_t)(v < 0 ? 0 : v);
}
template <typename T>
__host__ __device__ inline size_t mlp_out_index(const MlpArgs<T>& a, int z, int row, int ch) {
  if (a.tbQ > 0) return ((size_t)((row >> 6) * a.C + ch) * a.tbQ) * 128 + z * 64 + (row & 63);
  return ((size_t)z * a.M * a.C + (size_t)row * a.C + ch) * a.ld;
}
constexpr int mlp_param_count(int C, int H, int nlin) {
  return nlin == 1 ? 2 * C * 2 * C + 2 * C : (H * 2 * C + H) + (nlin - 2) * (H * H + H) + (2 * C * H + 2 * C);
}
template <typename T> int mlp_dispatch(const MlpArgs<T>&, bool backward, hipStream_t);
int cg_product_fwd(int R, int N, int C, int D1, int D2, int DO, int mode, int nnz, const int* row_ptr, const int* col, const double* coef,
                   const double* x1, const double* x2, double* out, hipStream_t st);
int cg_product_bwd(int R, int N, int C, int D1, int D2, int DO, int mode, int nnz, const int* row_ptr, const int* col, const double* coef,
                   const double* x1, const double* x2, const double* g_out, double* g_x1, double* g_x2, hipStream_t st);
int mlp_mfma_dispatch(const MlpArgs<double>&, bool backward, hipStream_t);
int mlp_chain_dispatch(const MlpArgs<double>&, bool backward, hipStream_t);
int mlp_mfma_wide_dispatch(const MlpArgs<double>&, bool backward, hipStream_t);
inline int mlp_rows_per_workgroup(int M, int H) { return (H <= 48 && (M + 63) / 64 < 128) ? 16 : 64; }
inline int mlp_partial_rows(int M, int H) { const int r = mlp_rows_per_workgroup(M, H); return (M + r - 1) / r; }

template <typename T>
struct MixArgs {
  int rows, Cin, Cout, d;
  const T* w;
  const T* x;
  T* y;
  const T* g_y;
  T* g_x;
  T* part;
};
template <typename T> int mix_fwd(const MixArgs<T>&, hipStream_t);
template <typename T> int mix_bwd(const MixArgs<T>&, hipStream_t);
int mix_partial_rows(int rows);

struct GenArgs {
  int B, N, C, Q;
  const double* X;
  const double* p;
  const uint8_t* mask;
  const double *ra, *rb, *rc, *w0, *b0, *w1, *b1;
  double* U;
  const double* gU;
  double* gX;
  double* g_p;
  double* part_rad;
  double* gbuf;
  int flags;
  int tb;
};
__host__ __device__ inline size_t feat_index(bool tb, size_t plane, int C, int Qx, int n, int c, int q, int z) {
  return tb ? ((size_t)((n >> 6) * C + c) * Qx + q) * 128 + z * 64 + (n & 63) : (size_t)z * plane + ((size_t)n * C + c) * Qx + q;
}
// ... 77 lines not shown
```

### lgn-autoencoder_amd/csrc/step.hip

```cpp
#include <stdlib.h>

#include <algorithm>
#include <vector>

#include "net.hpp"
#include "../../include/lgn_amd.h"

namespace lgn {
namespace {

inline size_t r16(size_t n) { return (n + 15) & ~size_t(15); }

struct Bump {
  double* base;
  size_t off = 0;
  double* here() const { return base ? base + off : nullptr; }
  double* take(size_t n) {
    double* p = here();
    off += r16(n);
    return p;
  }
};

struct Deferred {
// ... 195 lines not shown
  if (!loss || loss->kind == LGN_LOSS_CHAMFER) return 0;
  if (int rc = check_desc(d)) return rc;
  al = AssignLoss{loss->kind, loss->abs_coord, loss->polar_coord, loss->scale, assignment, status};
  const int Nd = dec_nodes(*d), CL = d->dec_channels[d->n_levels];
  if (int rc = check_assign_loss(al, Nd)) return rc;
  LGN_CHECK_ARG(d->jet_loss_scale == 0.0, "step: jet_loss_scale=%g with loss kind %d: the jet-feature term is a Chamfer option "
                "(--chamfer-jet-features)", d->jet_loss_scale, loss->kind);
  const size_t need = assign_loss_lds_bytes(Nd, CL);
  LGN_CHECK_ARG(need <= LGN_LDS_LIMIT, "step: the assignment-loss stage at N=%d needs %zu B of LDS (> %d)", Nd, need, LGN_LDS_LIMIT);
  *out = &al;
  return 0;
}

struct NetBuf {
  double *s[5], *v[5], *smix[4], *ag0[4], *ag1[4];
  double* hsave[4];
  double* sep[4];
};
void carve_net(Bump& b, const lgn_net_desc& d, bool dec, size_t BN, bool last_mlp_bwd, NetBuf& n) {
  const int* ch = dec ? d.dec_channels : d.enc_channels;
  const int L = d.n_levels;
  for (int l = 0; l <= L; ++l) {
    n.s[l] = b.take(2 * BN * ch[l]);
    n.v[l] = b.take(8 * BN * ch[l]);
  }
  for (int l = 0; l < L; ++l) {
    n.smix[l] = b.take(2 * BN * ch[l + 1]);
    n.ag0[l] = b.take(4 * BN * ch[l]);
    n.ag1[l] = b.take(16 * BN * ch[l]);
    n.sep[l] = dec ? b.take((size_t)d.B * sep_sums_doubles(ch[l])) : nullptr;
    const size_t hs = (last_mlp_bwd || l + 1 < L) && BN <= mlp_save_max_rows()
                          ? mlp_saved_doubles((int)BN, d.mlp_hidden_mul * 2 * ch[l + 1], d.mlp_nlin) : 0;
    n.hsave[l] = hs ? b.take(hs) : nullptr;
  }
}

struct BwdScratch {
  double *gs[2], *gv[2];
  double *gsmix, *g_ag;
  double *zeros_s, *g_p, *g_lat_s, *tail_cnt;
  size_t zero_doubles;
  double* zero0() const { return tail_cnt < zeros_s ? tail_cnt : zeros_s; }
  double* tot[4];
  double* parts;
  size_t parts_size;
};
void carve_level_grads(Bump& b, size_t BN, int cmax, BwdScratch& k) {
  for (int q = 0; q < 2; ++q) {
    k.gs[q] = b.take(2 * BN * cmax);
    k.gv[q] = b.take(8 * BN * cmax);
  }
  k.gsmix = b.take(2 * BN * cmax);
  k.g_ag = b.take(20 * BN * cmax);
}
inline size_t tot_doubles(int C, bool dec) { return rad_partial_size(C, dec) + 16; }

size_t net_parts(const lgn_net_desc& d, bool dec, int N) {
  const int* ch = dec ? d.dec_channels : d.enc_channels;
  int rm, rr;
  level_bwd_partial_rows(d.B, N, dec, d.flags, &rm, &rr);
  size_t sum = 0;
  for (int l = 0; l < d.n_levels; ++l) {
    const int H = d.mlp_hidden_mul * 2 * ch[l + 1];
    sum += r16((size_t)rm * 4 * ch[l + 1] * 5 * ch[l]) + r16((size_t)rr * rad_partial_size(ch[l], dec)) +
           r16((size_t)mlp_partial_rows(d.B * (dec ? dec_nodes(d) : N), H) * mlp_param_count(ch[l + 1], H, d.mlp_nlin));
  }
  return sum + end_parts(d, dec, N, rm > d.B ? rm : d.B);
}

struct InputStage {
  const double *w0, *w1;
  double* z1 = nullptr;
  size_t z1n = 0;
  double* z2 = nullptr;
  size_t z2n = 0;
};
struct LossStage {
  const double *wo1, *target;
  double scale;
  int method;
  double jscale;
  double *recon, *loss_part, *g_v, *wpart;
};

int levels_fwd(const lgn_net_desc& d, bool dec, const double* P, const int64_t* off, NetBuf& n, const double* pos, const uint8_t* mask,
               hipStream_t st, const InputStage* in0, const LossStage* loss, bool eval, bool last_scalars) {
  const Slots S{d.n_levels, d.mlp_nlin};
  const int* ch = dec ? d.dec_channels : d.enc_channels;
  for (int l = 0; l < d.n_levels; ++l) {
    auto p = [&](int slot) { return P + off[slot]; };
    LevelArgs<double> a{d.B, d.N, ch[l], ch[l + 1], n.s[l], n.v[l], pos, mask,
                        p(S.rad(dec, l, 0)), p(S.rad(dec, l, 1)), p(S.rad(dec, l, 2)), p(S.rad(dec, l, 3)), p(S.rad(dec, l, 4)),
                        p(S.rad(dec, l, 5)), p(S.rad(dec, l, 6)), p(S.mix(dec, l, 0)), p(S.mix(dec, l, 1)),
                        n.ag0[l], n.ag1[l], n.smix[l], n.v[l + 1]};
    if (l == 0 && !dec && in0) {
      a.in_w0 = in0->w0; a.in_w1 = in0->w1; a.in_s = n.s[0]; a.in_v = n.v[0];
      a.z1 = in0->z1; a.z1n = in0->z1n; a.z2 = in0->z2; a.z2n = in0->z2n;
    }
    if (l + 1 == d.n_levels && dec && loss) {
      a.loss_wo1 = loss->wo1; a.loss_target = loss->target; a.loss_scale = loss->scale; a.loss_real = loss->method;
      a.loss_jscale = loss->jscale; a.loss_recon = loss->recon;
      a.loss_part = loss->loss_part; a.loss_gv = loss->g_v; a.loss_wpart = loss->wpart;
    }
    a.flags = d.flags;
    if (dec && !eval && level_dec_rebuilds(d.N, d.flags)) a.sep_sums = n.sep[l];
    const bool no_mlp = l + 1 == d.n_levels && (!last_scalars || (eval && dec));
    a.dead_scalars = no_mlp && !(d.flags & LVL_LIVE_SCALARS);
    LGN_TRY(eval ? level_fwd_eval(a, dec, st) : level_fwd_dispatch<double>(a, dec, st));
    if (no_mlp) break;
    MlpArgs<double> m = level_mlp_args(d, dec, l, P, off);
    m.s_in = n.smix[l]; m.s_out = n.s[l + 1];
    m.h_saved = n.hsave[l]; m.h_rows = mlp_saved_rows(m.M);
    LGN_TRY(mlp_dispatch<double>(m, false, st));
  }
  return 0;
}

int levels_bwd(const lgn_net_desc& d, bool dec, const double* P, double* G, const int64_t* off, const NetBuf& n, const double* pos,
               const uint8_t* mask, BwdScratch& w, Deferred& dq, RadFinJob& fin, int& cur, bool has_s_grad, hipStream_t st,
               bool* in0_done = nullptr) {
  const Slots S{d.n_levels, d.mlp_nlin};
  const int* ch = dec ? d.dec_channels : d.enc_channels;
  const int BN = d.B * d.N;
  for (int l = d.n_levels - 1; l >= 0; --l) {
    auto p = [&](int slot) { return P + off[slot]; };
    auto g = [&](int slot) { return G + off[slot]; };
    const int C = ch[l], CO = ch[l + 1];
    const double* g_smix = w.zeros_s;
    if (has_s_grad) {
      MlpArgs<double> m = level_mlp_args(d, dec, l, P, off);
      m.s_in = n.smix[l]; m.g_out = w.gs[cur]; m.g_in = w.gsmix;
      m.h_saved = n.hsave[l];
      m.h_rows = mlp_saved_rows(BN);
      m.psize = mlp_param_count(CO, m.H, m.nlin);
      DQ_TAKE(m.part, (size_t)mlp_partial_rows(BN, m.H) * m.psize);
      LGN_TRY(mlp_dispatch<double>(m, true, st));
      dq.add(m.part, mlp_partial_rows(BN, m.H), m.psize, 0, m.psize, g(S.mlp(dec, l, 0)));
      g_smix = w.gsmix;
    }
    int rm, rr;
    level_bwd_partial_rows(d.B, d.N, dec, d.flags, &rm, &rr);
    const int nmix = 4 * CO * 5 * C, nrad = rad_partial_size(C, dec);
    DQ_NEW(part_mix, (size_t)rm * nmix);
    DQ_NEW(part_rad, (size_t)rr * nrad);
    const int nxt = cur ^ 1;
    LevelBwdArgs<double> a{d.B, d.N, C, CO, n.s[l], n.v[l], pos, mask,
                           p(S.rad(dec, l, 0)), p(S.rad(dec, l, 1)), p(S.rad(dec, l, 2)), p(S.rad(dec, l, 3)), p(S.rad(dec, l, 4)),
                           p(S.rad(dec, l, 5)), p(S.rad(dec, l, 6)), p(S.mix(dec, l, 0)), p(S.mix(dec, l, 1)), n.ag0[l], n.ag1[l],
                           g_smix, w.gv[cur], w.g_ag, w.gs[nxt], w.gv[nxt], dec ? w.g_p : nullptr, part_mix, part_rad};
    const bool dead_s = !has_s_grad && !(d.flags & LVL_LIVE_SCALARS);
    a.dead_scalars = dead_s;
    const bool carry_in0 = !dec && l == 0 && in0_done && level_bwd_carries_input(d.N, d.flags);
    const RowLayout rin = enc_input_rows(1, C);
    if (carry_in0) { DQ_TAKE(a.part_in0, (size_t)rm * rin.width); }
    a.flags = d.flags;
    if (dec && level_dec_rebuilds(d.N, d.flags)) a.sep_sums = n.sep[l];
    LGN_TRY(level_bwd_dispatch<double>(a, dec, st));
    if (carry_in0) {
      rin.add(dq, a.part_in0, rm, G, off);
      *in0_done = true;
    }
    if (dead_s) dq.add(nullptr, 0, 0, 0, nmix / 2, g(S.mix(dec, l, 0)));
    else dq.add(part_mix, rm, nmix, 0, nmix / 2, g(S.mix(dec, l, 0)));
    dq.add(part_mix, rm, nmix, nmix / 2, nmix / 2, g(S.mix(dec, l, 1)));
    if (dec) {
      dq.add(part_rad, rr, nrad, 0, C, g(S.rad(dec, l, 4)));
      dq.add(part_rad, rr, nrad, C, C, g(S.rad(dec, l, 6)));
    } else {
      double* tot = w.tot[l];
      dq.add(part_rad, rr, nrad, 0, nrad, tot);
      fin.it[fin.n++] = RadFinJob::Item{tot, C, p(S.rad(dec, l, 0)), p(S.rad(dec, l, 1)), p(S.rad(dec, l, 2)), p(S.rad(dec, l, 3)),
                                        p(S.rad(dec, l, 5)), g(S.rad(dec, l, 0)), g(S.rad(dec, l, 1)), g(S.rad(dec, l, 2)),
                                        g(S.rad(dec, l, 3)), g(S.rad(dec, l, 4)), g(S.rad(dec, l, 5)), g(S.rad(dec, l, 6))};
    }
    cur = nxt;
    has_s_grad = true;
  }
  return 0;
}

int encoder_fwd(const lgn_net_desc& d, const double* P, const int64_t* off, const double* p4, const uint8_t* mask, const double* xs,
                NetBuf& n, double* lat_s, double* lat_v, int* idx, hipStream_t st, const InputStage* ride, bool with_latent = true,
                bool eval = false, bool last_scalars = true) {
  const Slots S{d.n_levels, d.mlp_nlin};
  const int L = d.n_levels;
  const int* ce = d.enc_channels;
  if (!ride) LGN_TRY(enc_input_fwd(d.B, d.N, ce[0], in_K(d), p4, xs, P + off[0], P + off[1], n.s[0], n.v[0], st));
  LGN_TRY(levels_fwd(d, false, P, off, n, p4, mask, st, ride, nullptr, eval, last_scalars));
  if (with_latent)
    LGN_TRY(enc_latent_fwd(d.B, d.N, ce[L], d.tau_s, d.tau_v, d.latent_pool, last_scalars ? n.s[L] : nullptr, n.v[L], P + off[S.out0(false)],
                           P + off[S.out0(false) + 1], lat_s, lat_v, idx, st));
  return 0;
}

int encoder_bwd(const lgn_net_desc& d, const double* P, double* G, const int64_t* off, const double* p4, const uint8_t* mask,
                const double* xs, const NetBuf& n, const int* idx, const double* g_lat_s, const double* g_lat_v, BwdScratch& k, int cur,
                Deferred& dq, RadFinJob& fin, hipStream_t st, bool ride_in0, bool last_scalars = true, const JunctionBwd* jb = nullptr) {
  const Slots S{d.n_levels, d.mlp_nlin};
  const int L = d.n_levels, B = d.B, N = d.N, K = in_K(d);
  const int* ce = d.enc_channels;
  {
    const RowLayout rl = enc_latent_rows(d, N, ce[L]);
    const double *sL = last_scalars ? n.s[L] : nullptr, *wl0 = P + off[S.out0(false)], *wl1 = P + off[S.out0(false) + 1];
    DQ_NEW(parte, (size_t)B * rl.width);
    if (jb)
      LGN_TRY(junction_bwd(B, N, jb->C0, jb->Tin, jb->lat_v, jb->wg1, jb->w1, jb->pdec, jb->g_p, jb->g_s0, jb->g_v0, const_cast<double*>(g_lat_v),
                           jb->part_dec, ce[L], d.tau_s, d.tau_v, d.latent_pool, sL, n.v[L], wl0, wl1, g_lat_s ? g_lat_s : k.g_lat_s, idx,
                           k.gs[cur], k.gv[cur], parte, st));
    else
      LGN_TRY(enc_latent_bwd(B, N, ce[L], d.tau_s, d.tau_v, d.latent_pool, sL, n.v[L], wl0, wl1, g_lat_s ? g_lat_s : k.g_lat_s, g_lat_v, idx,
                             k.gs[cur], k.gv[cur], parte, st));
    rl.add(dq, parte, B, G, off);
  }
  bool in0_done = false;
  LGN_TRY(levels_bwd(d, false, P, G, off, n, p4, mask, k, dq, fin, cur, g_lat_s != nullptr, st, ride_in0 ? &in0_done : nullptr));
  if (!in0_done) {
    const RowLayout ri = enc_input_rows(K, ce[0]);
    DQ_NEW(part, (size_t)B * ri.width);
    LGN_TRY(enc_input_bwd(B, N, ce[0], K, p4, xs, k.gs[cur], k.gv[cur], part, st));
    ri.add(dq, part, B, G, off);
  }
  return 0;
}

int decoder_fwd(const lgn_net_desc& d, const double* P, const int64_t* off, const double* lat_v, NetBuf& n, double* pdec, hipStream_t st,
                bool with_input = true, const LossStage* loss = nullptr, bool eval = false, bool last_scalars = true) {
  if (with_input)
    LGN_TRY(dec_input_fwd(d.B, d.N, d.dec_channels[0], dec_tin(d), lat_v, P + off[1], P + off[2], P + off[3], pdec, n.s[0], n.v[0], st));
  return levels_fwd(d, true, P, off, n, pdec, nullptr, st, nullptr, loss, eval, last_scalars);
}

int decoder_bwd(const lgn_net_desc& d, const double* P, double* G, const int64_t* off, const double* lat_v, const NetBuf& n,
                const double* pdec, double* g_lat_v, BwdScratch& k, int& cur, Deferred& dq, RadFinJob& fin, hipStream_t st,
                double** part_in = nullptr) {
  const int B = d.B, N = d.N, C0 = d.dec_channels[0], Tin = dec_tin(d);
  LGN_TRY(levels_bwd(d, true, P, G, off, n, pdec, nullptr, k, dq, fin, cur, false, st));
  const RowLayout ri = dec_input_rows(C0, N, Tin);
  DQ_NEW(part, (size_t)B * ri.width);
  if (part_in) *part_in = part;
  else LGN_TRY(dec_input_bwd(B, N, C0, Tin, lat_v, P + off[1], P + off[3], pdec, k.g_p, k.gs[cur], k.gv[cur], g_lat_v, part, st));
  ri.add(dq, part, B, G, off);
  return 0;
}

inline bool is_generic(const lgn_net_desc& d, bool dec) { return (dec ? d.dec_tables[0] : d.enc_tables[0]) != nullptr; }

struct GenGeom {
  const int *ch, *Q, *qs, *qv;
  const lgn_local_tables* const* tab;
};
inline GenGeom geom(const lgn_net_desc& d, bool dec) {
  return dec ? GenGeom{d.dec_channels, d.dec_Q, d.dec_qs, d.dec_qv, d.dec_tables}
             : GenGeom{d.enc_channels, d.enc_Q, d.enc_qs, d.enc_qv, d.enc_tables};
}

inline bool is_static(const lgn_net_desc& d, bool dec) {
  const GenGeom g = geom(d, dec);
  if (d.N > 32) return false;
  for (int l = 0; l < d.n_levels; ++l)
    if (!g.tab[l] || g.tab[l]->static_kind == 0) return false;
  return !(d.flags & LGN_NET_NO_STATIC);
}
inline bool is_sep_fused(const lgn_net_desc& d, bool dec) {
  return dec && is_static(d, dec) && !(d.flags & (LGN_NET_DEC_PAIRWISE | LGN_NET_DEC_UNFUSED));
}
inline size_t tb_doubles(const lgn_net_desc& d, int C, int Qx) { return (size_t)(((size_t)d.B * d.N + 63) / 64) * C * Qx * 128; }

int check_generic(const lgn_net_desc& d, bool dec) {
  const GenGeom g = geom(d, dec);
  for (int l = 0; l < d.n_levels; ++l) {
    LGN_CHECK_ARG(g.tab[l], "table-driven network: level %d has no tables (every level needs one)", l);
    LGN_CHECK_ARG(g.tab[l]->n_w > 0 && g.tab[l]->n_rows > 0, "table-driven network: empty tables at level %d", l);
  }
  for (int l = 0; l <= d.n_levels; ++l)
    LGN_CHECK_ARG(g.Q[l] >= 5 && g.Q[l] <= 64 && g.qs[l] >= 0 && g.qs[l] < g.Q[l] && g.qv[l] >= 0 && g.qv[l] + 4 <= g.Q[l],
                  "table-driven network: bad component layout at level %d (Q=%d qs=%d qv=%d)", l, g.Q[l], g.qs[l], g.qv[l]);
  LGN_CHECK_ARG(g.Q[0] == 5, "table-driven network: the input level carries (1,1) and (0,0) only (Q=5), got %d", g.Q[0]);
  return 0;
}

struct GenAct {
  double *s0, *v0;
  double *X[5], *U[4], *smix[4];
  double* wp[4];
  double* tbl[4];
  double* pc;
  double *sL, *vL;
  double* pdec;
  int* idx;
  size_t total;
};
GenAct carve_gen_act(const lgn_net_desc& d, bool dec, double* base) {
  GenAct a{};
  Bump b{base};
  const GenGeom g = geom(d, dec);
  const size_t BN = (size_t)d.B * d.N;
  const int L = d.n_levels;
  a.s0 = b.take(2 * BN * g.ch[0]);
  a.v0 = b.take(8 * BN * g.ch[0]);
  const bool tb = is_static(d, dec);
  const bool sep = is_sep_fused(d, dec);
  for (int l = 0; l <= L; ++l) a.X[l] = b.take(tb ? tb_doubles(d, g.ch[l], g.Q[l]) : 2 * BN * g.ch[l] * g.Q[l]);
  a.pc = sep ? b.take(8 * BN) : nullptr;
  for (int l = 0; l < L; ++l) {
    a.U[l] = sep ? nullptr : b.take(tb ? tb_doubles(d, g.ch[l], 5 * g.Q[l]) : 10 * BN * g.ch[l] * g.Q[l]);
    a.tbl[l] = sep ? b.take((size_t)d.B * g.ch[l] * g.Q[l] * SEP_TBL_STRIDE) : nullptr;
    a.smix[l] = b.take(2 * BN * g.ch[l + 1]);
    a.wp[l] = tb ? b.take(local_static_packed_doubles(g.tab[l]->static_kind, g.ch[l], g.ch[l + 1])) : nullptr;
  }
  a.sL = b.take(2 * BN * g.ch[L]);
  a.vL = b.take(8 * BN * g.ch[L]);
  if (dec) a.pdec = b.take(8 * BN);
// ... 326 lines not shown
  carve_net(b, d, dec, BN, true, a.n);
  if (dec) a.pdec = b.take(8 * BN);
  else a.idx = reinterpret_cast<int*>(b.take(pool_idx_doubles(d)));
  a.total = b.off;
  return a;
}

struct NetScratch : BwdScratch {
  size_t total;
};
NetScratch carve_scratch(const lgn_net_desc& d, bool dec, double* base) {
  NetScratch s{};
  Bump b{base};
  const size_t BN = (size_t)d.B * d.N;
  const int L = d.n_levels;
  const int* ch = dec ? d.dec_channels : d.enc_channels;
  const int cmax = *std::max_element(ch, ch + L + 1);
  {
    const size_t z0 = b.off;
    s.tail_cnt = b.take(8);
    s.zeros_s = b.take(2 * BN * cmax);
    s.g_p = b.take(dec ? 8 * BN : 0);
    s.g_lat_s = b.take(dec ? 0 : lat_s_doubles(d));
    s.zero_doubles = b.off - z0;
  }
  carve_level_grads(b, BN, cmax, s);
  for (int l = 0; l < L; ++l) s.tot[l] = b.take(tot_doubles(ch[l], dec));
  s.parts_size = net_parts(d, dec, d.N);
  s.parts = b.take(s.parts_size);
  s.total = b.off;
  return s;
}

struct StepNets {
  NetBuf enc, dec;
  double *lat_s, *lat_v, *pdec;
  int* idx;
};
struct Work : StepNets {
  double* g_lat_v;
  BwdScratch k;
  size_t total;
};
Work carve(const lgn_net_desc& d, double* base) {
  Work w{};
  Bump b{base};
  const int Nd = dec_nodes(d), Nmax = d.N > Nd ? d.N : Nd;
  const size_t BN = (size_t)d.B * Nmax;
  const int L = d.n_levels;
  const int cmax = std::max(*std::max_element(d.enc_channels, d.enc_channels + L + 1), *std::max_element(d.dec_channels, d.dec_channels + L + 1));
  carve_net(b, d, false, (size_t)d.B * d.N, false, w.enc);
  carve_net(b, d, true, (size_t)d.B * Nd, false, w.dec);
  w.lat_s = b.take(lat_s_doubles(d));
  w.lat_v = b.take(lat_v_doubles(d));
  w.g_lat_v = b.take(lat_v_doubles(d));
  w.pdec = b.take(8 * BN);
  BwdScratch& k = w.k;
  carve_level_grads(b, BN, cmax, k);
  {
    const size_t z0 = b.off;
    k.zeros_s = b.take(2 * BN * cmax);
    k.g_p = b.take(8 * BN);
    k.g_lat_s = b.take(lat_s_doubles(d));
    k.tail_cnt = b.take(8);
    k.zero_doubles = b.off - z0;
  }
  w.idx = reinterpret_cast<int*>(b.take(pool_idx_doubles(d)));
  for (int l = 0; l < L; ++l) k.tot[l] = b.take(tot_doubles(d.enc_channels[l], false));
  for (int l = 0; l < L; ++l) b.take(tot_doubles(d.dec_channels[l], true));
  k.parts_size = net_parts(d, false, d.N) + net_parts(d, true, Nd);
  k.parts = b.take(k.parts_size);
  w.total = b.off;
  return w;
}

int autoencoder_fwd(const lgn_net_desc& d, const lgn_net_desc& dd, const double* params, const int64_t* enc_off, const int64_t* dec_off,
                    const double* p4, const uint8_t* mask, const double* in_scalars, StepNets& w, const InputStage& ride,
                    const LossStage* loss, bool eval, bool keep_s, hipStream_t st) {
  const Slots S{d.n_levels, d.mlp_nlin};
  const int L = d.n_levels;
  const bool split = step_is_split(d);
  LGN_TRY(encoder_fwd(d, params, enc_off, p4, mask, in_scalars, w.enc, w.lat_s, w.lat_v, w.idx, st, split ? nullptr : &ride,
                      split, eval, keep_s));
  if (!split)
    LGN_TRY(junction_fwd(d.B, d.N, d.enc_channels[L], d.tau_s, d.tau_v, d.latent_pool, keep_s ? w.enc.s[L] : nullptr, w.enc.v[L],
                         params + enc_off[S.out0(false)], params + enc_off[S.out0(false) + 1], w.lat_s, w.lat_v, w.idx, d.dec_channels[0],
                         params + dec_off[1], params + dec_off[2], params + dec_off[3], w.pdec, w.dec.s[0], w.dec.v[0], st));
  return decoder_fwd(dd, params, dec_off, w.lat_v, w.dec, w.pdec, st, split, loss, eval, false);
}

struct GenStep {
  GenAct ea, da;
  GenScratch es, ds;
  double *lat_s, *lat_v, *g_lat_v;
  size_t total;
};
GenStep carve_gen_step(const lgn_net_desc& d, double* base) {
  GenStep g{};
  Bump b{base};
  g.ea = carve_gen_act(d, false, b.here()); b.take(g.ea.total);
  g.da = carve_gen_act(d, true, b.here()); b.take(g.da.total);
  g.es = carve_gen_scratch(d, false, b.here()); b.take(g.es.total);
  g.ds = carve_gen_scratch(d, true, b.here()); b.take(g.ds.total);
  g.lat_s = b.take(lat_s_doubles(d));
  g.lat_v = b.take(lat_v_doubles(d));
  g.g_lat_v = b.take(lat_v_doubles(d));
  g.total = b.off;
  return g;
}

int gen_autoencoder_fwd(const lgn_net_desc& d, const double* params, const int64_t* enc_off, const int64_t* dec_off, const double* p4,
                        const uint8_t* mask, GenAct& ea, GenAct& da, double* lat_s, double* lat_v, hipStream_t st) {
  const Slots S{d.n_levels, d.mlp_nlin};
  LGN_TRY(gen_encoder_fwd(d, params, enc_off, p4, mask, ea, lat_s, lat_v, st, nullptr, false));
  LGN_TRY(junction_fwd(d.B, d.N, d.enc_channels[d.n_levels], d.tau_s, d.tau_v, d.latent_pool, ea.sL, ea.vL, params + enc_off[S.out0(false)],
                       params + enc_off[S.out0(false) + 1], lat_s, lat_v, ea.idx, d.dec_channels[0], params + dec_off[1], params + dec_off[2],
                       params + dec_off[3], da.pdec, da.s0, da.v0, st));
  return gen_decoder_fwd(d, params, dec_off, lat_v, da, st, false);
}

int gen_step_fwd_bwd(const lgn_net_desc& d, const double* params, double* grads, long long n_params, const int64_t* enc_off,
                     const int64_t* dec_off, const double* p4, const double* target, const uint8_t* mask, double* workspace,
                     long long workspace_doubles, double* recon, double* loss_part, hipStream_t st, const StepTailArgs* tail,
                     const AssignLoss* al) {
  LGN_CHECK_ARG(is_generic(d, false) && is_generic(d, true), "step: encoder and decoder must both be table-driven (or both fused)");
  if (int rc = check_generic(d, false)) return rc;
  if (int rc = check_generic(d, true)) return rc;
  GenStep g = carve_gen_step(d, workspace);
  LGN_CHECK_ARG((long long)g.total <= workspace_doubles, "step: workspace holds %lld doubles, this configuration needs %zu",
                workspace_doubles, g.total);
  if (int rc = check_mlp_contiguous(d, false, enc_off)) return rc;
  if (int rc = check_mlp_contiguous(d, true, dec_off)) return rc;
  const Slots S{d.n_levels, d.mlp_nlin};
  const int L = d.n_levels, B = d.B, N = d.N, CL = d.dec_channels[L];
  LGN_TRY(zero_ranges(grads, (size_t)n_params, g.es.zero0, g.es.zero_doubles, g.ds.zero0, g.ds.zero_doubles, st));
  LGN_TRY(gen_autoencoder_fwd(d, params, enc_off, dec_off, p4, mask, g.ea, g.da, g.lat_s, g.lat_v, st));
  Deferred dq(g.ds.parts, g.ds.parts_size);
  RadFinJob fin{};
  {
    const RowLayout ro = dec_output_rows(d, CL);
    DQ_NEW(part, (size_t)B * ro.width);
    if (al)
      LGN_TRY(dec_output_assign_loss(B, N, CL, g.da.vL, params + dec_off[S.out0(true) + 1], target, d.get_real, *al, recon, loss_part,
                                     g.ds.gv, part, st));
    else
      LGN_TRY(dec_output_loss(B, N, CL, g.da.vL, params + dec_off[S.out0(true) + 1], target, 1.0, d.get_real, d.jet_loss_scale, recon,
                              loss_part, g.ds.gv, part, st));
    ro.add(dq, part, B, grads, dec_off);
  }
  std::vector<UnpackJob> post;
  double* part_in = nullptr;
  LGN_TRY(gen_decoder_bwd(d, params, grads, dec_off, g.lat_v, g.da, g.g_lat_v, g.ds, dq, fin, post, st, &part_in));
  const int Tin = dec_tin(d), C0d = d.dec_channels[0];
  const JunctionBwd jb{C0d, Tin, g.lat_v, params + dec_off[1], params + dec_off[3], g.da.pdec, g.ds.g_p, g.ds.gs, g.ds.gv, part_in};
  if (!post.empty() || !is_static(d, false) || !is_static(d, true)) {
    LGN_TRY(dec_input_bwd(B, N, C0d, Tin, g.lat_v, params + dec_off[1], params + dec_off[3], g.da.pdec, g.ds.g_p, g.ds.gs, g.ds.gv, g.g_lat_v,
                          part_in, st));
    LGN_TRY(dq.flush(st));
    LGN_TRY(run_unpack_jobs(post, st));
    LGN_TRY(gen_encoder_bwd(d, params, grads, enc_off, p4, mask, g.ea, nullptr, g.g_lat_v, g.es, st));
    if (tail) LGN_TRY(finalize_tail(*tail, st));
    return 0;
  }
  LGN_TRY(gen_encoder_bwd(d, params, grads, enc_off, p4, mask, g.ea, nullptr, g.g_lat_v, g.es, st, nullptr, &dq, &fin, &jb));
  return end_step(dq, fin, grads, n_params, nullptr, d.flags, tail, st);
}

int step_fwd_bwd(const lgn_net_desc* dp, const double* params, double* grads, long long n_params, const int64_t* enc_off,
                 const int64_t* dec_off, const double* p4, const double* target, const uint8_t* mask, const double* in_scalars,
                 double* workspace, long long workspace_doubles, double* recon, double* loss_part, void* stream,
                 const StepTailArgs* tail, const AssignLoss* al = nullptr) {
// ... 226 lines not shown
  if (int rc = check_mlp_contiguous(*d, false, off)) return rc;
  LGN_TRY(zero_grads_and_block(grads, (size_t)n_params, sc.zero0(), sc.zero_doubles, st));
  Deferred dq(sc.parts, sc.parts_size);
  RadFinJob fin{};
  LGN_TRY(encoder_bwd(*d, params, grads, off, p4, mask, in_scalars, a.n, a.idx, g_lat_s, g_lat_v, sc, 0, dq, fin, st,
                      in_K(*d) == 1));
  return finish_reductions(dq, fin, grads, n_params, nullptr, d->flags, st);
}

int lgn_decoder_fwd_f64(const lgn_net_desc* d, const double* params, const int64_t* off, const double* lat_v, double* act,
                        long long act_doubles, double* recon, void* stream) {
  if (int rc = check_desc(d)) return rc;
  LGN_CHECK_ARG(params && off && lat_v && act && recon, "decoder_fwd: null pointer");
  hipStream_t st = (hipStream_t)stream;
  const int CL = d->dec_channels[d->n_levels];
  const double* wo1 = params + off[Slots{d->n_levels, d->mlp_nlin}.out0(true) + 1];
  if (is_generic(*d, true)) {
    if (int rc = check_generic(*d, true)) return rc;
    GenAct ga = carve_gen_act(*d, true, act);
    LGN_CHECK_ARG((long long)ga.total <= act_doubles, "decoder_fwd: activation buffer holds %lld doubles, needs %zu", act_doubles, ga.total);
    LGN_TRY(gen_decoder_fwd(*d, params, off, lat_v, ga, st));
    return dec_output_fwd(d->B, d->N, CL, ga.vL, wo1, recon, st);
  }
  NetAct a = carve_act(*d, true, act);
  LGN_CHECK_ARG((long long)a.total <= act_doubles, "decoder_fwd: activation buffer holds %lld doubles, needs %zu", act_doubles, a.total);
  LGN_TRY(decoder_fwd(*d, params, off, lat_v, a.n, a.pdec, st));
  return dec_output_fwd(d->B, d->N, CL, a.n.v[d->n_levels], wo1, recon, st);
}

int lgn_decoder_bwd_f64(const lgn_net_desc* d, const double* params, double* grads, long long n_params, const int64_t* off,
                        const double* lat_v, const double* act, long long act_doubles, const double* g_recon, double* g_lat_v,
                        double* scratch, long long scratch_doubles, void* stream) {
  if (int rc = check_desc(d)) return rc;
  LGN_CHECK_ARG(params && grads && off && lat_v && act && g_recon && g_lat_v && scratch && n_params > 0, "decoder_bwd: null pointer");
  hipStream_t st = (hipStream_t)stream;
  const int B = d->B, N = d->N, CL = d->dec_channels[d->n_levels];
  const double* wo1 = params + off[Slots{d->n_levels, d->mlp_nlin}.out0(true) + 1];
  const RowLayout ro = dec_output_rows(*d, CL);
  RadFinJob fin{};
  if (is_generic(*d, true)) {
    if (int rc = check_generic(*d, true)) return rc;
    GenAct ga = carve_gen_act(*d, true, const_cast<double*>(act));
    GenScratch gs = carve_gen_scratch(*d, true, scratch);
    LGN_CHECK_ARG((long long)ga.total <= act_doubles && (long long)gs.total <= scratch_doubles,
                  "decoder_bwd: buffers hold %lld / %lld doubles, need %zu / %zu", act_doubles, scratch_doubles, ga.total, gs.total);
    if (int rc = check_mlp_contiguous(*d, true, off)) return rc;
    LGN_TRY(zero_grads_and_block(grads, (size_t)n_params, gs.zero0, gs.zero_doubles, st));
    Deferred dq(gs.parts, gs.parts_size);
    DQ_NEW(part, (size_t)B * ro.width);
    LGN_TRY(dec_output_bwd(B, N, CL, ga.vL, wo1, g_recon, gs.gv, part, st));
    ro.add(dq, part, B, grads, off);
    std::vector<UnpackJob> post;
    LGN_TRY(gen_decoder_bwd(*d, params, grads, off, lat_v, ga, g_lat_v, gs, dq, fin, post, st));
    LGN_TRY(dq.flush(st));
    return run_unpack_jobs(post, st);
  }
  NetAct a = carve_act(*d, true, const_cast<double*>(act));
  NetScratch sc = carve_scratch(*d, true, scratch);
  LGN_CHECK_ARG((long long)a.total <= act_doubles && (long long)sc.total <= scratch_doubles,
                "decoder_bwd: buffers hold %lld / %lld doubles, need %zu / %zu", act_doubles, scratch_doubles, a.total, sc.total);
  if (int rc = check_mlp_contiguous(*d, true, off)) return rc;
  LGN_TRY(zero_grads_and_block(grads, (size_t)n_params, sc.zero0(), sc.zero_doubles, st));
  Deferred dq(sc.parts, sc.parts_size);
  int cur = 0;
  DQ_NEW(part, (size_t)B * ro.width);
  LGN_TRY(dec_output_bwd(B, N, CL, a.n.v[d->n_levels], wo1, g_recon, sc.gv[cur], part, st));
  ro.add(dq, part, B, grads, off);
  LGN_TRY(decoder_bwd(*d, params, grads, off, lat_v, a.n, a.pdec, g_lat_v, sc, cur, dq, fin, st));
  return finish_reductions(dq, fin, grads, n_params, nullptr, d->flags, st);
}

int lgn_step_param_slots(const lgn_net_desc* d, int decoder) {
  if (check_desc(d)) return -1;
  return Slots{d->n_levels, d->mlp_nlin}.count(decoder != 0);
}

long long lgn_encoder_end_lds_bytes(int N, int C0, int K, int CL, int Ts, int Tv, int pool) {
  return pool_valid(pool) ? (long long)encoder_end_lds_bytes(N, C0, K < 1 ? 1 : K, CL, Ts, Tv, pool) : -1;
}
long long lgn_decoder_end_lds_bytes(int N, int C0, int Tin, int CL) { return (long long)decoder_end_lds_bytes(N, C0, Tin, CL); }
long long lgn_junction_lds_bytes(int N, int CL, int Ts, int Tv, int pool, int C0) {
  return pool_valid(pool) ? (long long)junction_lds_bytes(N, CL, Ts, Tv, pool, C0) : -1;
}

long long lgn_step_workspace_doubles(const lgn_net_desc* d) {
  if (check_desc(d) || check_latent_match(*d)) return -1;
  if (is_generic(*d, false) || is_generic(*d, true)) {
    if (check_generic(*d, false) || check_generic(*d, true)) return -1;
    return (long long)carve_gen_step(*d, nullptr).total;
  }
  return (long long)carve(*d, nullptr).total;
}

int lgn_step_fwd_bwd_f64(const lgn_net_desc* d, const double* params, double* grads, long long n_params, const int64_t* enc_off,
                         const int64_t* dec_off, const double* p4, const double* target, const uint8_t* mask, const double* in_scalars,
                         double* workspace, long long workspace_doubles, double* recon, double* loss_part, const lgn_loss_desc* loss,
                         int* assignment, int* status, void* stream) {
  AssignLoss al;
  const AssignLoss* alp;
  if (int rc = plan_assign_loss(d, loss, assignment, status, al, &alp)) return rc;
  return step_fwd_bwd(d, params, grads, n_params, enc_off, dec_off, p4, target, mask, in_scalars, workspace, workspace_doubles, recon,
                      loss_part, stream, nullptr, alp);
}

int lgn_step_train_f64(const lgn_net_desc* d, double* params, double* grads, long long n_params, const int64_t* enc_off,
                       const int64_t* dec_off, const double* p4, const double* target, const uint8_t* mask, const double* in_scalars,
                       double* workspace, long long workspace_doubles, double* recon, double* loss_part, int n_loss, double l1_lambda,
                       double* adam_m, double* adam_v, long long* step_dev, double lr, double beta1, double beta2, double eps,
                       int do_adam, double* loss_out, const lgn_loss_desc* loss, int* assignment, int* status, void* stream) {
  AssignLoss al;
  const AssignLoss* alp;
  if (int rc = plan_assign_loss(d, loss, assignment, status, al, &alp)) return rc;
  LGN_CHECK_ARG(loss_out && n_loss > 0, "step_train: null pointer");
  LGN_CHECK_ARG(!do_adam || (adam_m && adam_v && step_dev), "step_train: Adam state missing");
  const StepTailArgs tail{params, grads, (long)n_params, adam_m, adam_v, reinterpret_cast<long*>(step_dev), l1_lambda, lr, beta1, beta2,
                          eps, do_adam, loss_part, n_loss, loss_out, 0, nullptr};
  return step_fwd_bwd(d, params, grads, n_params, enc_off, dec_off, p4, target, mask, in_scalars, workspace, workspace_doubles, recon,
                      loss_part, stream, &tail, alp);
}

int lgn_step_finalize_f64(double* params, double* grads, long long n_params, const double* loss_part, int n_loss, double l1_lambda,
                          double* adam_m, double* adam_v, long long* step_dev, double lr, double beta1, double beta2, double eps,
                          int do_adam, double* loss_out, void* stream) {
  LGN_CHECK_ARG(params && grads && loss_part && loss_out && n_params > 0 && n_loss > 0, "step_finalize: null pointer");
  LGN_CHECK_ARG(!do_adam || (adam_m && adam_v && step_dev), "step_finalize: Adam state missing");
  hipStream_t st = (hipStream_t)stream;
  LGN_TRY(finalize_step(params, grads, (long)n_params, loss_part, n_loss, l1_lambda, adam_m, adam_v, reinterpret_cast<long*>(step_dev),
                        lr, beta1, beta2, eps, do_adam, loss_out, st));
  return 0;
}

int lgn_step_train_opt_f64(const lgn_net_desc* d, double* params, double* grads, long long n_params, const int64_t* enc_off,
                           const int64_t* dec_off, const double* p4, const double* target, const uint8_t* mask, const double* in_scalars,
                           double* workspace, long long workspace_doubles, double* recon, double* loss_part, int n_loss,
                           const lgn_optim_desc* opt, double* state_m, double* state_v, long long* step_dev, int do_step,
                           double* loss_out, const lgn_loss_desc* loss, int* assignment, int* status, void* stream) {
  AssignLoss al;
  const AssignLoss* alp;
  if (int rc = plan_assign_loss(d, loss, assignment, status, al, &alp)) return rc;
  LGN_CHECK_ARG(loss_out && n_loss > 0, "step_train_opt: null pointer");
  StepTailArgs tail{};
  if (int rc = optim_tail(opt, params, grads, n_params, state_m, state_v, step_dev, do_step, loss_part, n_loss, loss_out, tail))
    return rc;
  return step_fwd_bwd(d, params, grads, n_params, enc_off, dec_off, p4, target, mask, in_scalars, workspace, workspace_doubles,
                      recon, loss_part, stream, &tail, alp);
}

int lgn_step_finalize_opt_f64(double* params, double* grads, long long n_params, const double* loss_part, int n_loss,
                              const lgn_optim_desc* opt, double* state_m, double* state_v, long long* step_dev, int do_step,
                              double* loss_out, void* stream) {
  LGN_CHECK_ARG(params && grads && loss_part && loss_out && n_params > 0 && n_loss > 0, "step_finalize_opt: null pointer");
  StepTailArgs tail{};
  if (int rc = optim_tail(opt, params, grads, n_params, state_m, state_v, step_dev, do_step, loss_part, n_loss, loss_out, tail))
    return rc;
  return finalize_step_opt(tail, (hipStream_t)stream);
}

long long lgn_eval_workspace_doubles(const lgn_net_desc* d) {
  if (check_desc(d)) return -1;
  return eval_workspace(*d);
}

int lgn_step_eval_f64(const lgn_net_desc* d, const double* params, const int64_t* enc_off, const int64_t* dec_off,
                      const double* p4_scaled, const double* p4_target, const uint8_t* mask, const double* in_scalars,
                      double* workspace, long long workspace_doubles, double* recon_real, double* lat_s, double* lat_v,
                      double* loss_part, double* loss_out, const lgn_loss_desc* loss, int* assignment, int* status, void* stream) {
// ... 9 lines not shown
```

### lgn-autoencoder_amd/lgn/_native.py

```python
from __future__ import annotations

import ctypes as C
import os
from typing import Optional, Sequence

import torch

_HERE = os.path.dirname(os.path.abspath(__file__))
LIB_PATH = os.environ.get("LGN_AMD_LIB") or os.path.join(_HERE, "_lib", "liblgn_amd.so")
ABI_VERSION = 19
FINALIZE_SCRATCH = 2048
FINALIZE_OPT_SCRATCH = 4096

_lib: Optional[C.CDLL] = None

_vp, _i, _ip = C.c_void_p, C.c_int, C.POINTER(C.c_int)

_SIGNATURES = {
    "lgn_level_fwd_f64": [_i] * 5 + [_vp] * 18,
    "lgn_level_bwd_partial_rows": [_i, _i, _i, _ip, _ip],
    "lgn_level_rad_partial_len": [_i, _i],
    "lgn_level_jet_split": [_i, _i],
    "lgn_cg_product_fwd_f64": [_i] * 8 + [_vp] * 7,
    "lgn_cg_product_bwd_f64": [_i] * 8 + [_vp] * 9,
# ... 3 lines not shown
    "lgn_cgmlp_fwd_f64": [_i] * 5 + [_vp] * 5,
    "lgn_cgmlp_partial_rows": [_i, _i],
    "lgn_cgmlp_bwd_f64": [_i] * 5 + [_vp] * 6 + [_i, _vp],
    "lgn_mixreps_fwd_f64": [_i] * 4 + [_vp] * 4,
    "lgn_chamfer_f64": [_i] * 3 + [_vp] * 2 + [_i] + [_vp] * 4,
    "lgn_mixreps_partial_rows": [_i],
    "lgn_mixreps_bwd_f64": [_i] * 4 + [_vp] * 6,
}


class LocalTables(C.Structure):
    _fields_ = [("n_rows", C.c_int), ("n_out", C.c_int), ("n_w", C.c_int), ("n_terms", C.c_int), ("n_u", C.c_int),
                ("n_x", C.c_int), ("n_units", C.c_int), ("static_kind", C.c_int)] + [
        (name, C.c_void_p) for name in ("row_ptr", "t_type", "t_a", "t_b", "t_coef", "out_dim", "out_nblk", "out_row0", "out_q0",
                                        "out_w0", "u_ptr", "u_row", "u_coef", "x_ptr", "x_row", "x_other", "x_coef")] + [("h_out_w0", C.c_int * 8)]


_tp = C.POINTER(LocalTables)


_POOL_OPS = {"min": 0, "max": 1, "mean": 2, "average": 2}


def pool_code(map_to_latent: str):
    m = map_to_latent.lower()
    if m == "mix":
        return 1 | (3 << 4)
    if "&" in m and "+" in m:
        return None
    avg = "+" in m
    ops = m.split("+") if avg else m.split("&")
    if not 1 <= len(ops) <= 4 or any(o not in _POOL_OPS for o in ops):
        return None
    code = len(ops) | (int(avg) << 3)
    for i, o in enumerate(ops):
        code |= _POOL_OPS[o] << (4 + 2 * i)
    return code


def end_stages_fit(encoder=None, decoder=None, junction: bool = False) -> bool:
    L = lib()
    need = 0
    if encoder is not None:
        code = pool_code(encoder.map_to_latent)
        if code is None:
            return False
        n = encoder.num_input_particles
        ch = encoder.num_channels
        ts, tv = encoder.tau_latent[(0, 0)], encoder.tau_latent[(1, 1)]
        need = max(need, L.lgn_encoder_end_lds_bytes(n, ch[0], max(1, encoder.tau_input_scalars), ch[-1], ts, tv, code))
        if junction and decoder is not None:
            need = max(need, L.lgn_junction_lds_bytes(n, ch[-1], ts, tv, code, decoder.num_channels[0]))
    if decoder is not None:
        ch = decoder.num_channels
        need = max(need, L.lgn_decoder_end_lds_bytes(decoder.num_output_particles, ch[0], decoder.tau_latent_vectors, ch[-1]))
    return 0 <= need <= LDS_LIMIT


def pool_blocks(code: int) -> int:
    if code == 0:
        return 2
    return 1 if (code >> 3) & 1 else code & 7


class NetDesc(C.Structure):
    _fields_ = [("B", C.c_int), ("N", C.c_int), ("n_levels", C.c_int), ("enc_channels", C.c_int * 5),
                ("dec_channels", C.c_int * 5), ("tau_s", C.c_int), ("tau_v", C.c_int), ("mlp_hidden_mul", C.c_int),
                ("mlp_nlin", C.c_int), ("tau_v_in", C.c_int),
                ("enc_tables", _tp * 4), ("dec_tables", _tp * 4),
                ("enc_Q", C.c_int * 5), ("enc_qs", C.c_int * 5), ("enc_qv", C.c_int * 5),
                ("dec_Q", C.c_int * 5), ("dec_qs", C.c_int * 5), ("dec_qv", C.c_int * 5), ("flags", C.c_int),
                ("activation", C.c_int), ("n_in_scalars", C.c_int), ("latent_pool", C.c_int), ("dec_N", C.c_int),
                ("get_real", C.c_int), ("jet_loss_scale", C.c_double)]

    def __init__(self, *a, **kw):
        super().__init__(*a, **kw)
        self.flags = net_flags()


NET_NO_STATIC = 1
_NET_FLAG_ENV = {"LGN_AMD_NO_STATIC": 1, "LGN_AMD_DEC_PAIRWISE": 2, "LGN_AMD_LEVEL_V2": 4, "LGN_AMD_MLP_V1": 8,
                 "LGN_AMD_MOMENTS_V1": 16, "LGN_AMD_BWD_ORDERED": 64, "LGN_AMD_LIVE_SCALARS": 4096, "LGN_AMD_SPLIT_TAIL": 128, "LGN_AMD_DEC_UNFUSED": 256, "LGN_AMD_MOMENTS_SPLIT": 512,
                 "LGN_AMD_MLP_BWD1": 1024, "LGN_AMD_MLP_FULLTILE": 2048,
                 "LGN_AMD_DEC_STORE_AG": 16384}
ACTIVATIONS = {"leakyrelu": 0, "relu": 1, "elu": 2, "sigmoid": 3, "logsigmoid": 4, "atan": 5}


def activation_id(name: str) -> int:
    try:
        return ACTIVATIONS[name.lower()]
    except KeyError:
        raise ValueError(f"Activation function {name} not implemented!") from None


def net_flags() -> int:
    return sum(bit for name, bit in _NET_FLAG_ENV.items() if os.environ.get(name, "") == "1")


class LossDesc(C.Structure):
    _fields_ = [("kind", C.c_int), ("abs_coord", C.c_int), ("polar_coord", C.c_int), ("scale", C.c_double)]


class OptimDesc(C.Structure):
    _fields_ = [("kind", C.c_int), ("l1_lambda", C.c_double), ("l2_lambda", C.c_double), ("lr", C.c_double), ("eps", C.c_double),
                ("beta1", C.c_double), ("beta2", C.c_double), ("alpha", C.c_double), ("momentum", C.c_double)]


OPT_ADAM, OPT_RMSPROP = 0, 1
LOSS_CHAMFER, LOSS_MSE, LOSS_HUNGARIAN = 0, 1, 2
ASSIGN_NMAX = 192
_dp = C.POINTER(NetDesc)
_lp = C.POINTER(LossDesc)
_op = C.POINTER(OptimDesc)
_ll = C.c_longlong
_d = C.c_double
_SIGNATURES.update({
    "lgn_moments_fwd_f64": [_i] * 5 + [_vp] * 12,
    "lgn_moments_bwd_f64": [_i] * 5 + [_vp] * 16,
    "lgn_local_fwd_f64": [_i] * 5 + [_tp] + [_vp] * 5,
    "lgn_local_partial_rows": [_i],
    "lgn_local_fwd_static_f64": [_i] * 4 + [_vp] * 3 + [_ip] + [_vp] * 3 + [_i, _vp],
    "lgn_local_bwd_static_f64": [_i] * 4 + [_vp] * 3 + [_ip] + [_vp] * 8,
    "lgn_local_bwd_f64": [_i] * 5 + [_tp] + [_vp] * 8,
    "lgn_step_param_slots": [_dp, _i],
    "lgn_step_fwd_bwd_f64": [_dp, _vp, _vp, _ll, _vp, _vp, _vp, _vp, _vp, _vp, _vp, _ll, _vp, _vp, _lp, _vp, _vp, _vp],
    "lgn_encoder_fwd_f64": [_dp, _vp, _vp, _vp, _vp, _vp, _vp, _ll, _vp, _vp, _vp],
    "lgn_encoder_bwd_f64": [_dp, _vp, _vp, _ll, _vp, _vp, _vp, _vp, _vp, _ll, _vp, _vp, _vp, _ll, _vp],
    "lgn_decoder_fwd_f64": [_dp, _vp, _vp, _vp, _vp, _ll, _vp, _vp],
    "lgn_decoder_bwd_f64": [_dp, _vp, _vp, _ll, _vp, _vp, _vp, _ll, _vp, _vp, _vp, _ll, _vp],
    "lgn_step_finalize_f64": [_vp, _vp, _ll, _vp, _i, _d, _vp, _vp, _vp, _d, _d, _d, _d, _i, _vp, _vp],
    "lgn_step_train_f64": [_dp, _vp, _vp, _ll, _vp, _vp, _vp, _vp, _vp, _vp, _vp, _ll, _vp, _vp, _i, _d, _vp, _vp, _vp, _d, _d, _d, _d, _i,
                           _vp, _lp, _vp, _vp, _vp],
    "lgn_step_finalize_opt_f64": [_vp, _vp, _ll, _vp, _i, _op, _vp, _vp, _vp, _i, _vp, _vp],
    "lgn_step_train_opt_f64": [_dp, _vp, _vp, _ll, _vp, _vp, _vp, _vp, _vp, _vp, _vp, _ll, _vp, _vp, _i, _op, _vp, _vp, _vp, _i, _vp, _lp,
                               _vp, _vp, _vp],
    "lgn_step_eval_f64": [_dp, _vp, _vp, _vp, _vp, _vp, _vp, _vp, _vp, _ll, _vp, _vp, _vp, _vp, _vp, _lp, _vp, _vp, _vp],
    "lgn_anomaly_scores_f64": [_vp] * 4 + [_i] * 3 + [_vp] * 4,
    "lgn_linear_sum_assignment_f64": [_vp, _i, _i, _vp, _vp, _vp],
    "lgn_hungarian_mse_f64": [_i, _i, _vp, _vp, _i, _i, _i, _d] + [_vp] * 5,
    "lgn_recon_analysis_f64": [_vp, _vp] + [_i] * 4 + [_vp] * 11,
    "lgn_match_rel_err_f64": [_vp] * 6 + [_i, _i] + [_vp] * 5,
    "lgn_histogram_f64": [_vp, _ll, _i, _i, _vp, _ip, _i, _vp, _vp, _vp, _vp, _i, _vp],
    "lgn_stage_batch_f64": [_vp] * 3 + [_i] * 4 + [_d, _i, _i] + [_vp] * 6,
    "lgn_denormalize_f64": [_vp] * 3 + [_i, _i] + [_vp] * 3,
    "lgn_stage_gather_f64": [_vp] * 3 + [_ll, _vp, _ll, _vp] + [_i] * 3 + [_d, _i, _i] + [_vp] * 7,
    "lgn_epoch_collect_f64": [_vp] * 3 + [_ll, _i, _i, C.POINTER(_vp), C.POINTER(_vp), _ip, _vp],
    "lgn_epoch_reset": [_vp] * 4,
    "lgn_roc_auc_f64": [_vp, _ll, _i, _i] + [_vp] * 9 + [_ll, _vp],
    "lgn_emd_f64": [_vp, _vp, _i, _i, _i, _d] + [_vp] * 6 + [_ll, _vp],
    "lgn_emd_relative_f64": [_vp, _vp, _i, _i, _vp, _vp, _vp, _ll, _vp],
    "lgn_emd_grad_f64": [_vp, _vp, _i, _i, _i, _d] + [_vp] * 8 + [_ll, _vp],
    "lgn_emd_relative_grad_f64": [_vp, _vp, _i, _i] + [_vp] * 5 + [_ll, _vp],
    "lgn_emd_debug_max_augmentations": [_ip, _i],
    "lgn_column_stats_f64": [_vp, _ll, _i, _i, _vp, _i, _d, _i] + [_vp] * 5 + [_ll, _vp],
    "lgn_hist_fwhm_f64": [_vp, _i, _vp, _i, _ip, _i, _vp, _vp],
    "lgn_jet_images_f64": [_vp, _vp, _i, _i, _i, _i, _d, _i, _vp, _vp, _vp, _ll, _vp],
    "lgn_transform_jets_f64": [_vp] * 4 + [_i] * 4 + [_vp] * 3,
    "lgn_rep_deviation_f64": [_i] * 3 + [C.POINTER(_vp)] * 3 + [_ip] * 3 + [_vp] * 3 + [_ll, _vp],
})
EPOCH_MAX_COLLECT, EPOCH_BAD_INDEX = 4, 1
NORM_NONE, NORM_COMPONENT_MAX, NORM_OVERALL_MAX, NORM_JET_E = 0, 1, 2, 3


_LL_SIGNATURES = {
    "lgn_step_workspace_doubles": [_dp],
    "lgn_eval_workspace_doubles": [_dp],
    "lgn_net_workspace_doubles": [_dp, _i, _i],
    "lgn_moments_scratch_doubles": [_i, _i, _i, _i],
    "lgn_local_static_packed_doubles": [_i, _i, _i],
    "lgn_encoder_end_lds_bytes": [_i] * 7,
    "lgn_decoder_end_lds_bytes": [_i] * 4,
    "lgn_junction_lds_bytes": [_i] * 6,
    "lgn_assign_loss_lds_bytes": [_i, _i],
    "lgn_roc_workspace_bytes": [_ll, _i],
    "lgn_emd_workspace_bytes": [_i, _i],
    "lgn_emd_lds_bytes": [_i],
    "lgn_column_stats_workspace_bytes": [_ll, _i],
    "lgn_jet_images_workspace_bytes": [_i, _i],
    "lgn_rep_deviation_workspace_bytes": [_i, _i, _i, _ip, _ip, _ip],
}
ROC_TILE, ROC_MAX_COLS = 2048, 65535
ROC_NONFINITE, ROC_SINGLE_CLASS, ROC_BAD_LABEL, ROC_NAN = 1, 2, 4, 8
EMD_NMAX = 191
EMD_INVALID, EMD_EMPTY, EMD_ITER, EMD_INFEASIBLE = 1, 2, 4, 8
HIST_MAX_EDGES, HIST_MAX_COLS = 1025, 16
STATS_TILE, STATS_MAX_COLS, STATS_EMPTY, STATS_NONFINITE = 2048, 16, 1, 2
STAT_NAMES = ("median", "IQR", "first_quartile", "third_quartile", "IDR", "MAD", "mean", "max", "min", "abs_min", "std_dev", "skew",
              "kurtosis", "FWHM", "abs_mean", "abs_mean_within_iqr", "abs_mean_within_idr", "q10", "q90")
STATS_COUNT = len(STAT_NAMES)
JET_IMAGE_MAX_NPIX, JET_IMAGE_PARTS = 64, 512
EQUI_TILE, EQUI_MAX_PARTS = 256, 64
LDS_LIMIT = 160 * 1024
EXPORTED_SYMBOLS = ["lgn_abi_version", "lgn_last_error"] + list(_LL_SIGNATURES) + list(_SIGNATURES)


def lib() -> C.CDLL:
    global _lib
    if _lib is None:
        if not os.path.exists(LIB_PATH):
            raise RuntimeError(
                f"liblgn_amd.so not found at {LIB_PATH}. Build it with `python -c 'import __graft_entry__ as g; "
                "g.build()'` or `make -C lgn-autoencoder_amd/csrc`. There is no CPU fallback.")
        l = C.CDLL(LIB_PATH)
        l.lgn_abi_version.restype = C.c_int
        l.lgn_last_error.restype = C.c_char_p
        got = l.lgn_abi_version()
        if got != ABI_VERSION:
# ... 266 lines not shown
```

Baseline: 1.132 million.

## Fold encoder-decoder junction stage into first decoder level forward kernel

Runs the latent pooling and decoder input stages inside the first separable decoder level forward kernel when the LDS budget allows, instead of launching a separate junction kernel. The decoder's first-level node features and momenta are written straight into LDS, which skips a kernel launch and a global round trip of the decoder inputs. The cost is a larger LDS footprint for that kernel, which may lower occupancy, plus extra block-level syncs. An env flag restores the separate launch.

```diff
diff --git a/include/lgn_amd.h b/include/lgn_amd.h
--- a/include/lgn_amd.h
+++ b/include/lgn_amd.h
@@ -157,6 +157,7 @@
 long long lgn_encoder_end_lds_bytes(int N, int C0, int K, int CL, int Ts, int Tv, int pool);
 long long lgn_decoder_end_lds_bytes(int N, int C0, int Tin, int CL);
 long long lgn_junction_lds_bytes(int N, int CL, int Ts, int Tv, int pool, int C0);
+int lgn_junction_rides(const lgn_net_desc* d);
 
 int lgn_step_param_slots(const lgn_net_desc* d, int decoder);
 long long lgn_step_workspace_doubles(const lgn_net_desc* d);
diff --git a/lgn-autoencoder_amd/csrc/level.hpp b/lgn-autoencoder_amd/csrc/level.hpp
--- a/lgn-autoencoder_amd/csrc/level.hpp
+++ b/lgn-autoencoder_amd/csrc/level.hpp
@@ -12,6 +12,7 @@
 constexpr int LVL_MOMENTS_SPLIT = 512;
 constexpr int LVL_LIVE_SCALARS = 4096;
 constexpr int LVL_DEC_STORE_AG = 16384;
+constexpr int LVL_JUNCTION_LAUNCH = 32768;
 constexpr int LVL_BWD_ORDERED = 64;
 int level_flags_from_env();
 
@@ -48,6 +49,20 @@
   int flags = 0;
   int dead_scalars = 0;
   T* sep_sums = nullptr;
+  const T* jn_wl0 = nullptr;
+  const T* jn_wl1 = nullptr;
+  const T* jn_s = nullptr;
+  const T* jn_v = nullptr;
+  const T* jn_wg1 = nullptr;
+  const T* jn_w0 = nullptr;
+  const T* jn_w1 = nullptr;
+  T* jn_lat_s = nullptr;
+  T* jn_lat_v = nullptr;
+  int* jn_idx = nullptr;
+  T* jn_pdec = nullptr;
+  T* jn_s0 = nullptr;
+  T* jn_v0 = nullptr;
+  int jn_CL = 0, jn_Ts = 0, jn_Tv = 0, jn_pool = 0;
 };
 constexpr int sep_sums_doubles(int C) { return 20 * C + 8; }
 
diff --git a/lgn-autoencoder_amd/csrc/level_fwd2.hip b/lgn-autoencoder_amd/csrc/level_fwd2.hip
--- a/lgn-autoencoder_amd/csrc/level_fwd2.hip
+++ b/lgn-autoencoder_amd/csrc/level_fwd2.hip
@@ -77,6 +77,32 @@
           a.in_v[plane_s * 4 + ge * 4 + m] = d[6 + m];
         }
       }
+    }
+  } else if (DEC && SEP && a.jn_wl0) {
+    if constexpr (DEC && SEP) {
+      const int CL = a.jn_CL, Ts = a.jn_Ts, Tv = a.jn_Tv, pool = a.jn_pool, Tin = pool_blocks(pool) * Tv;
+      double* lat_lds = agl;
+      double* dec_lds = lat_lds + lat_fwd_doubles(N, CL, Ts, Tv, pool);
+      LatentStage ls;
+      DecInFwdStage ds;
+      ls.issue(B, N, CL, Ts, Tv, a.jn_s, a.jn_v, a.jn_wl0, a.jn_wl1, pool);
+      ds.issue(B, N, C, Tin, nullptr, a.jn_wg1, a.jn_w0, a.jn_w1, false);
+      const int nw2 = 2 * CO * 5 * C, ew = tid < nw2 ? tid : 0;
+      const double w0v = a.wm0[ew], w1v = a.wm1[ew];
+      ls.commit(lat_lds, false);
+      ds.commit(dec_lds);
+      if (tid < nw2) {
+        wm[tid] = w0v;
+        wm[nw2 + tid] = w1v;
+      }
+      for (int e = tid + nthr; e < nw2; e += nthr) {
+        wm[e] = a.wm0[e];
+        wm[nw2 + e] = a.wm1[e];
+      }
+      __syncthreads();
+      enc_latent_fwd_body<true>(B, N, CL, Ts, Tv, pool, a.jn_lat_s, a.jn_lat_v, a.jn_idx, lat_lds, dec_lds + 2 * N * Tin);
+      __syncthreads();
+      dec_input_fwd_body<true>(B, N, C, Tin, a.jn_pdec, a.jn_s0, a.jn_v0, dec_lds, pj, nd, F::NS);
     }
   } else {
     JetRegs<double> jr;
@@ -495,6 +521,16 @@
   }
 }
 
+static size_t junction_ride_lds_bytes(int N, int C, int CO, int CL, int Ts, int Tv, int pool) {
+  const size_t head = (((size_t)N * node_stride(C) + 1) & ~size_t(1)) + (size_t)N * 8 + 4 * (size_t)CO * 5 * C;
+  return sizeof(double) * (head + lat_fwd_doubles(N, CL, Ts, Tv, pool) + dec_in_fwd_doubles(N, C, pool_blocks(pool) * Tv));
+}
+bool level_fwd_carries_junction(int N, int C, int CO, int CL, int Ts, int Tv, int pool, int flags) {
+  if (N < 1 || N > 40 || (flags & (LVL_DEC_PAIRWISE | LVL_LEVEL_V2 | LVL_JUNCTION_LAUNCH))) return false;
+  if (!pool_valid(pool) || pool_is_mix(pool)) return false;
+  return junction_ride_lds_bytes(N, C, CO, CL, Ts, Tv, pool_canon(pool)) <= 78 * 1024;
+}
+
 template <int C, bool DEC, bool SEP, bool TRAIN, bool NOS>
 static int launch_level_fwd2(const LevelArgs<double>& a, hipStream_t stream) {
   using F = Fwd2<C, DEC>;
@@ -514,6 +550,14 @@
     LGN_CHECK_ARG(DEC && SEP && a.N <= 40 && !wide && a.loss_target && a.loss_recon && a.loss_part && (!TRAIN || (a.loss_gv && a.loss_wpart)),
                   "level_fwd: the loss rides on the separable decoder forward of jets of <= 40 particles only");
     if (smem < dec_out_loss_bytes(a.N, a.CO)) smem = dec_out_loss_bytes(a.N, a.CO);
+  }
+  if (a.jn_wl0) {
+    LGN_CHECK_ARG(DEC && SEP && !wide && level_fwd_carries_junction(a.N, C, a.CO, a.jn_CL, a.jn_Ts, a.jn_Tv, a.jn_pool, 0) &&
+                      a.jn_pool == pool_canon(a.jn_pool) && a.jn_wl1 && a.jn_v && a.jn_wg1 && a.jn_w0 && a.jn_w1 && a.jn_lat_s && a.jn_lat_v &&
+                      a.jn_idx && a.jn_pdec && a.jn_s0 && a.jn_v0,
+                  "level_fwd: the stages between the networks ride on the separable decoder forward of jets of <= 40 particles only");
+    const size_t need = junction_ride_lds_bytes(a.N, C, a.CO, a.jn_CL, a.jn_Ts, a.jn_Tv, a.jn_pool);
+    if (smem < need) smem = need;
   }
   LGN_CHECK_ARG(!a.sep_sums || (DEC && SEP && TRAIN && a.N <= 40),
                 "level_fwd: only the separable decoder forward of a training step (N <= 40) leaves jet sums instead of the aggregate");
diff --git a/lgn-autoencoder_amd/csrc/net_dev.hpp b/lgn-autoencoder_amd/csrc/net_dev.hpp
--- a/lgn-autoencoder_amd/csrc/net_dev.hpp
+++ b/lgn-autoencoder_amd/csrc/net_dev.hpp
@@ -1,5 +1,6 @@
 #pragma once
 #include "common.hpp"
+#include "net.hpp"
 
 namespace lgn {
 
@@ -290,4 +291,249 @@
   }
 }
 
-}
+__device__ __forceinline__ void cart_from_canon(const cx<double> (&c)[4], cx<double> (&p)[4]) {
+  p[0] = c[0];
+  p[1] = {(c[1].r - c[3].r) * NET_RSQRT2, (c[1].i - c[3].i) * NET_RSQRT2};
+  p[2] = {-(c[1].i + c[3].i) * NET_RSQRT2, (c[1].r + c[3].r) * NET_RSQRT2};
+  p[3] = c[2];
+}
+__device__ __forceinline__ cx<double> canon_cplx_m(const double* p, int m) {
+  if (m == 0) return {p[0], p[4]};
+  if (m == 2) return {p[3], p[7]};
+  const double sg = m == 1 ? 1.0 : -1.0;
+  return {(sg * p[1] + p[6]) * NET_RSQRT2, (sg * p[5] - p[2]) * NET_RSQRT2};
+}
+__device__ __forceinline__ double latent_norm4(const double* o) {
+#pragma clang fp contract(off)
+  return __builtin_fma(o[0], o[0], -__builtin_fma(o[3], o[3], __builtin_fma(o[1], o[1], o[2] * o[2])));
+}
+__device__ __forceinline__ cx<double> dec_in_cmul(cx<double> a, cx<double> b) {
+#pragma clang fp contract(off)
+  return {__builtin_fma(a.r, b.r, -(a.i * b.i)), __builtin_fma(a.i, b.r, a.r * b.i)};
+}
+
+__host__ __device__ inline size_t lat_y_doubles(int N, int Ts, int Tv, int pool = 0) {
+  return (size_t)(pool_is_mix(pool) ? 1 : N) * (2 * Ts + 8 * Tv);
+}
+__host__ __device__ inline size_t lat_fwd_doubles(int N, int C, int Ts, int Tv, int pool = 0) {
+  return lat_y_doubles(N, Ts, Tv, pool) + (size_t)N * C * 10 + 2 * (size_t)(Ts + Tv) * pool_mix_in(pool, N, C);
+}
+struct LatentStage {
+  StageRegs<2> sr, si;
+  StageRegs<4> vr, vi;
+  StageRegs<1> w0, w1;
+  const double *s0, *s1, *v0, *v1, *wl0, *wl1;
+  int N, C, Ts, Tv, K, NY, NS;
+  __device__ __forceinline__ void issue(int B, int N_, int C_, int Ts_, int Tv_, const double* __restrict__ s, const double* __restrict__ v,
+                                        const double* __restrict__ wl0_, const double* __restrict__ wl1_, int pool = 0) {
+    N = N_; C = C_; Ts = Ts_; Tv = Tv_; wl0 = wl0_; wl1 = wl1_; K = pool_mix_in(pool, N_, C_); NY = (int)lat_y_doubles(N_, Ts_, Tv_, pool);
+    const size_t pl = (size_t)B * N * C, j0 = (size_t)blockIdx.x * N * C;
+    NS = s ? N * C : 0;
+    s0 = s ? s + j0 : nullptr; s1 = s ? s + pl + j0 : nullptr; v0 = v + j0 * 4; v1 = v + (pl + j0) * 4;
+    vr.issue(v0, N * C * 4); vi.issue(v1, N * C * 4);
+    sr.issue(s0, NS); si.issue(s1, NS);
+    w0.issue(wl0, 2 * Ts * K); w1.issue(wl1, 2 * Tv * K);
+  }
+  __device__ __forceinline__ void commit(double* lds, bool zero_y) const {
+    double* sv = lds + NY;
+    double* w0l = sv + N * C * 10;
+    double* w1l = w0l + 2 * Ts * K;
+    if (zero_y)
+      for (int e = threadIdx.x; e < NY; e += BLOCK) lds[e] = 0.0;
+    vr.commit(v0, N * C * 4, [&](int e, double x) { sv[(e >> 2) * 10 + 2 + (e & 3)] = x; });
+    vi.commit(v1, N * C * 4, [&](int e, double x) { sv[(e >> 2) * 10 + 6 + (e & 3)] = x; });
+    if (NS) {
+      sr.commit(s0, NS, [&](int e, double x) { sv[e * 10] = x; });
+      si.commit(s1, NS, [&](int e, double x) { sv[e * 10 + 1] = x; });
+    } else {
+      for (int e = threadIdx.x; e < N * C; e += BLOCK) sv[e * 10] = sv[e * 10 + 1] = 0.0;
+    }
+    w0.commit(wl0, 2 * Ts * K, [&](int e, double x) { w0l[e] = x; });
+    w1.commit(wl1, 2 * Tv * K, [&](int e, double x) { w1l[e] = x; });
+  }
+};
+template <bool TO_LDS>
+__device__ __forceinline__ void enc_latent_fwd_body(int B, int N, int C, int Ts, int Tv, int pool, double* lat_s, double* lat_v, int* idx,
+                                                    double* lds, double* lat_l) {
+  const int b = blockIdx.x, TT = Ts + Tv;
+  const int P = pool_blocks(pool), PN = pool_n(pool);
+  bool need_mean = false;
+  for (int i = 0; i < PN; ++i) need_mean |= pool_op(pool, i) == LGN_POOL_MEAN;
+  const int YS = 2 * Ts + 8 * Tv;
+  double* y = lds;
+  const double* sv = y + N * YS;
+  const double* w0l = sv + N * C * 10;
+  const double* w1l = w0l + 2 * Ts * C;
+  STAMP(1);
+  for (int e = threadIdx.x; e < N * Tv; e += BLOCK) {
+    const int n = e / Tv, tv = e - n * Tv;
+    const double* x = sv + n * C * 10;
+    cx<double> acc[4] = {{0, 0}, {0, 0}, {0, 0}, {0, 0}}, pc[4];
+#pragma unroll 4
+    for (int c = 0; c < C; ++c) {
+      const cx<double> w = {w1l[tv * C + c], w1l[Tv * C + tv * C + c]};
+#pragma unroll
+      for (int m = 0; m < 4; ++m) cfma(acc[m], w, cx<double>{x[c * 10 + 2 + m], x[c * 10 + 6 + m]});
+    }
+    cart_from_canon(acc, pc);
+    double* o = y + n * YS + 2 * Ts + 8 * tv;
+#pragma unroll
+    for (int m = 0; m < 4; ++m) { o[m] = pc[m].r; o[4 + m] = pc[m].i; }
+  }
+  for (int e = threadIdx.x; e < N * Ts; e += BLOCK) {
+    const int n = e / Ts, t = e - n * Ts;
+    const double* x = sv + n * C * 10;
+    cx<double> acc = {0, 0};
+#pragma unroll 4
+    for (int c = 0; c < C; ++c) cfma(acc, cx<double>{w0l[t * C + c], w0l[Ts * C + t * C + c]}, cx<double>{x[c * 10], x[c * 10 + 1]});
+    y[n * YS + 2 * t] = acc.r;
+    y[n * YS + 2 * t + 1] = acc.i;
+  }
+  __syncthreads();
+  STAMP(2);
+  const int l8 = threadIdx.x & 7;
+  constexpr int NONE = 0x7fffffff;
+  for (int it = threadIdx.x >> 3; it < 2 * TT; it += BLOCK / 8) {
+    const int z = it / TT, t = it - z * TT;
+    int imin = NONE, imax = NONE;
+    double smin = 0, smax = 0;
+#pragma unroll 4
+    for (int n = l8; n < N; n += 8) {
+      double lo, hi;
+      if (t < Ts) {
+        const double val = y[n * YS + 2 * t + z];
+        lo = val;
+        hi = val * val;
+      } else {
+        const double* o = y + n * YS + 2 * Ts + 8 * (t - Ts) + 4 * z;
+        lo = hi = latent_norm4(o);
+      }
+      if (imin == NONE || lo < smin) { smin = lo; imin = n; }
+      if (imax == NONE || hi > smax) { smax = hi; imax = n; }
+    }
+#pragma unroll
+    for (int off = 4; off; off >>= 1) {
+      const double om = __shfl_xor(smin, off, 8), oM = __shfl_xor(smax, off, 8);
+      const int oi = __shfl_xor(imin, off, 8), oI = __shfl_xor(imax, off, 8);
+      if (oi != NONE && (imin == NONE || om < smin || (om == smin && oi < imin))) { smin = om; imin = oi; }
+      if (oI != NONE && (imax == NONE || oM > smax || (oM == smax && oI < imax))) { smax = oM; imax = oI; }
+    }
+    imin = __shfl(imin, 0, 8);
+    imax = __shfl(imax, 0, 8);
+    if (l8 < 2) idx[(((size_t)b * 2 + z) * TT + t) * 2 + l8] = l8 ? imax : imin;
+    const int nc = t < Ts ? 1 : 4, y0 = t < Ts ? 2 * t + z : 2 * Ts + 8 * (t - Ts) + 4 * z;
+    double mean[4] = {0, 0, 0, 0};
+    if (need_mean) {
+      for (int n = l8; n < N; n += 8)
+#pragma unroll
+        for (int m = 0; m < 4; ++m)
+          if (m < nc) mean[m] += y[n * YS + y0 + m];
+#pragma unroll
+      for (int off = 4; off; off >>= 1)
+#pragma unroll
+        for (int m = 0; m < 4; ++m) mean[m] += __shfl_xor(mean[m], off, 8);
+#pragma unroll
+      for (int m = 0; m < 4; ++m) mean[m] /= (double)N;
+    }
+    for (int k = l8; k < P * nc; k += 8) {
+      const int pb = k / nc, m = k - pb * nc;
+      auto pick = [&](int op) -> double {
+        if (op == LGN_POOL_MIN) return y[imin * YS + y0 + m];
+        if (op == LGN_POOL_MAX) return y[imax * YS + y0 + m];
+        return m == 0 ? mean[0] : (m == 1 ? mean[1] : (m == 2 ? mean[2] : mean[3]));
+      };
+      double val;
+      if (pool_avg(pool)) {
+        val = pick(pool_op(pool, 0));
+        for (int i = 1; i < PN; ++i) val += pick(pool_op(pool, i));
+        val /= (double)PN;
+      } else {
+        val = pick(pool_op(pool, pb));
+      }
+      if (t < Ts) {
+        lat_s[((size_t)z * B + b) * P * Ts + pb * Ts + t] = val;
+      } else {
+        const int tv = t - Ts;
+        lat_v[(((size_t)z * B + b) * P * Tv + pb * Tv + tv) * 4 + m] = val;
+        if constexpr (TO_LDS) lat_l[(pb * Tv + tv) * 8 + 4 * z + m] = val;
+      }
+    }
+  }
+}
+
+__host__ __device__ inline size_t dec_in_fwd_doubles(int N, int C, int Tin) {
+  return 2 * (size_t)N * Tin + (size_t)Tin * 8 + (size_t)N * 8 + 4 * (size_t)C;
+}
+struct DecInFwdStage {
+  StageRegs<4> wg;
+  StageRegs<1> a0, a1, lr, li;
+  const double *wg1, *w0, *w1, *l0, *l1;
+  int N, C, Tin;
+  bool with_lat;
+  __device__ __forceinline__ void issue(int B, int N_, int C_, int Tin_, const double* __restrict__ lat_v, const double* __restrict__ wg1_,
+                                        const double* __restrict__ w0_, const double* __restrict__ w1_, bool with_lat_) {
+    N = N_; C = C_; Tin = Tin_; wg1 = wg1_; w0 = w0_; w1 = w1_; with_lat = with_lat_;
+    wg.issue(wg1, 2 * N * Tin);
+    a0.issue(w0, 2 * C); a1.issue(w1, 2 * C);
+    if (with_lat) {
+      l0 = lat_v + (size_t)blockIdx.x * Tin * 4; l1 = lat_v + ((size_t)B + blockIdx.x) * Tin * 4;
+      lr.issue(l0, Tin * 4); li.issue(l1, Tin * 4);
+    }
+  }
+  __device__ __forceinline__ void commit(double* lds) const {
+    double* wgl = lds;
+    double* latl = wgl + 2 * N * Tin;
+    double* w01 = latl + Tin * 8 + N * 8;
+    wg.commit(wg1, 2 * N * Tin, [&](int e, double x) { wgl[e] = x; });
+    a0.commit(w0, 2 * C, [&](int e, double x) { w01[e] = x; });
+    a1.commit(w1, 2 * C, [&](int e, double x) { w01[2 * C + e] = x; });
+    if (with_lat) {
+      lr.commit(l0, Tin * 4, [&](int e, double x) { latl[(e >> 2) * 8 + (e & 3)] = x; });
+      li.commit(l1, Tin * 4, [&](int e, double x) { latl[(e >> 2) * 8 + 4 + (e & 3)] = x; });
+    }
+  }
+};
+template <bool TO_LEVEL = false>
+__device__ __forceinline__ void dec_input_fwd_body(int B, int N, int C, int Tin, double* pdec, double* s0, double* v0, double* lds,
+                                                   double* pj_l = nullptr, double* nd_l = nullptr, int NS = 0) {
+  const double* wgl = lds;
+  const double* latl = wgl + 2 * N * Tin;
+  double* cartl = const_cast<double*>(latl) + Tin * 8;
+  const double* w01 = cartl + N * 8;
+  const int b = blockIdx.x;
+  const size_t plp = (size_t)B * N * 4, pl = (size_t)B * N * C;
+  STAMP(3);
+  for (int e = threadIdx.x; e < N * 4; e += BLOCK) {
+    const int n = e >> 2, m = e & 3;
+    cx<double> acc = {0, 0};
+#pragma unroll 8
+    for (int t = 0; t < Tin; ++t)
+      cfma(acc, cx<double>{wgl[n * Tin + t], wgl[N * Tin + n * Tin + t]}, cx<double>{latl[t * 8 + m], latl[t * 8 + 4 + m]});
+    cartl[n * 8 + m] = acc.r;
+    cartl[n * 8 + 4 + m] = acc.i;
+  }
+  __syncthreads();
+  STAMP(4);
+  for (int e = threadIdx.x; e < N * 4; e += BLOCK) {
+    const cx<double> pc = canon_cplx_m(cartl + (e >> 2) * 8, e & 3);
+    pdec[(size_t)b * N * 4 + e] = pc.r;
+    pdec[plp + (size_t)b * N * 4 + e] = pc.i;
+    if constexpr (TO_LEVEL) { pj_l[(e >> 2) * 8 + (e & 3)] = pc.r; pj_l[(e >> 2) * 8 + 4 + (e & 3)] = pc.i; }
+  }
+  for (int e = threadIdx.x; e < N * C; e += BLOCK) {
+    const int c = e % C;
+    const double sr = w01[c] - w01[C + c], si = w01[C + c] + w01[c];
+    s0[(size_t)b * N * C + e] = sr;
+    s0[pl + (size_t)b * N * C + e] = si;
+    if constexpr (TO_LEVEL) { double* d = nd_l + (e / C) * NS + c * 10; d[0] = sr; d[1] = si; }
+  }
+  for (int e = threadIdx.x; e < N * C * 4; e += BLOCK) {
+    const int i = e >> 2, m = e & 3, n = i / C, c = i - n * C;
+    const cx<double> r = dec_in_cmul(cx<double>{w01[2 * C + c], w01[3 * C + c]}, canon_cplx_m(cartl + n * 8, m));
+    v0[(size_t)b * N * C * 4 + e] = r.r;
+    v0[pl * 4 + (size_t)b * N * C * 4 + e] = r.i;
+    if constexpr (TO_LEVEL) { double* d = nd_l + n * NS + c * 10; d[2 + m] = r.r; d[6 + m] = r.i; }
+  }
+}
+
+}
diff --git a/lgn-autoencoder_amd/csrc/net_kernels.hip b/lgn-autoencoder_amd/csrc/net_kernels.hip
--- a/lgn-autoencoder_amd/csrc/net_kernels.hip
+++ b/lgn-autoencoder_amd/csrc/net_kernels.hip
@@ -30,12 +30,6 @@
   gp[1] = {(g[1].r - g[3].r) * H, (g[1].i - g[3].i) * H};
   gp[2] = {-(g[1].i + g[3].i) * H, (g[1].r + g[3].r) * H};
   gp[3] = g[2];
-}
-__device__ __forceinline__ void cart_from_canon(const cx<double> (&c)[4], cx<double> (&p)[4]) {
-  p[0] = c[0];
-  p[1] = {(c[1].r - c[3].r) * H, (c[1].i - c[3].i) * H};
-  p[2] = {-(c[1].i + c[3].i) * H, (c[1].r + c[3].r) * H};
-  p[3] = c[2];
 }
 }
 
@@ -117,12 +111,6 @@
   }
 }
 
-__device__ __forceinline__ cx<double> canon_cplx_m(const double* p, int m) {
-  if (m == 0) return {p[0], p[4]};
-  if (m == 2) return {p[3], p[7]};
-  const double sg = m == 1 ? 1.0 : -1.0;
-  return {(sg * p[1] + p[6]) * H, (sg * p[5] - p[2]) * H};
-}
 __device__ __forceinline__ cx<double> canon_cplx_bwd_m(const double* g, int m) {
   if (m == 0) return {g[0], g[4]};
   if (m == 3) return {g[2], g[6]};
@@ -130,154 +118,6 @@
   return {-(g[5] + g[7]) * H, (g[1] + g[3]) * H};
 }
 
-__host__ __device__ inline size_t lat_y_doubles(int N, int Ts, int Tv, int pool = 0) {
-  return (size_t)(pool_is_mix(pool) ? 1 : N) * (2 * Ts + 8 * Tv);
-}
-__host__ __device__ inline size_t lat_fwd_doubles(int N, int C, int Ts, int Tv, int pool = 0) {
-  return lat_y_doubles(N, Ts, Tv, pool) + (size_t)N * C * 10 + 2 * (size_t)(Ts + Tv) * pool_mix_in(pool, N, C);
-}
-struct LatentStage {
-  StageRegs<2> sr, si;
-  StageRegs<4> vr, vi;
-  StageRegs<1> w0, w1;
-  const double *s0, *s1, *v0, *v1, *wl0, *wl1;
-  int N, C, Ts, Tv, K, NY, NS;
-  __device__ __forceinline__ void issue(int B, int N_, int C_, int Ts_, int Tv_, const double* __restrict__ s, const double* __restrict__ v,
-                                        const double* __restrict__ wl0_, const double* __restrict__ wl1_, int pool = 0) {
-    N = N_; C = C_; Ts = Ts_; Tv = Tv_; wl0 = wl0_; wl1 = wl1_; K = pool_mix_in(pool, N_, C_); NY = (int)lat_y_doubles(N_, Ts_, Tv_, pool);
-    const size_t pl = (size_t)B * N * C, j0 = (size_t)blockIdx.x * N * C;
-    NS = s ? N * C : 0;
-    s0 = s ? s + j0 : nullptr; s1 = s ? s + pl + j0 : nullptr; v0 = v + j0 * 4; v1 = v + (pl + j0) * 4;
-    vr.issue(v0, N * C * 4); vi.issue(v1, N * C * 4);
-    sr.issue(s0, NS); si.issue(s1, NS);
-    w0.issue(wl0, 2 * Ts * K); w1.issue(wl1, 2 * Tv * K);
-  }
-  __device__ __forceinline__ void commit(double* lds, bool zero_y) const {
-    double* sv = lds + NY;
-    double* w0l = sv + N * C * 10;
-    double* w1l = w0l + 2 * Ts * K;
-    if (zero_y)
-      for (int e = threadIdx.x; e < NY; e += BLOCK) lds[e] = 0.0;
-    vr.commit(v0, N * C * 4, [&](int e, double x) { sv[(e >> 2) * 10 + 2 + (e & 3)] = x; });
-    vi.commit(v1, N * C * 4, [&](int e, double x) { sv[(e >> 2) * 10 + 6 + (e & 3)] = x; });
-    if (NS) {
-      sr.commit(s0, NS, [&](int e, double x) { sv[e * 10] = x; });
-      si.commit(s1, NS, [&](int e, double x) { sv[e * 10 + 1] = x; });
-    } else {
-      for (int e = threadIdx.x; e < N * C; e += BLOCK) sv[e * 10] = sv[e * 10 + 1] = 0.0;
-    }
-    w0.commit(wl0, 2 * Ts * K, [&](int e, double x) { w0l[e] = x; });
-    w1.commit(wl1, 2 * Tv * K, [&](int e, double x) { w1l[e] = x; });
-  }
-};
-template <bool TO_LDS>
-__device__ __forceinline__ void enc_latent_fwd_body(int B, int N, int C, int Ts, int Tv, int pool, double* lat_s, double* lat_v, int* idx,
-                                                    double* lds, double* lat_l) {
-  const int b = blockIdx.x, TT = Ts + Tv;
-  const int P = pool_blocks(pool), PN = pool_n(pool);
-  bool need_mean = false;
-  for (int i = 0; i < PN; ++i) need_mean |= pool_op(pool, i) == LGN_POOL_MEAN;
-  const int YS = 2 * Ts + 8 * Tv;
-  double* y = lds;
-  const double* sv = y + N * YS;
-  const double* w0l = sv + N * C * 10;
-  const double* w1l = w0l + 2 * Ts * C;
-  STAMP(1);
-  for (int e = threadIdx.x; e < N * Tv; e += BLOCK) {
-    const int n = e / Tv, tv = e - n * Tv;
-    const double* x = sv + n * C * 10;
-    cx<double> acc[4] = {{0, 0}, {0, 0}, {0, 0}, {0, 0}}, pc[4];
-#pragma unroll 4
-    for (int c = 0; c < C; ++c) {
-      const cx<double> w = {w1l[tv * C + c], w1l[Tv * C + tv * C + c]};
-#pragma unroll
-      for (int m = 0; m < 4; ++m) cfma(acc[m], w, cx<double>{x[c * 10 + 2 + m], x[c * 10 + 6 + m]});
-    }
-    cart_from_canon(acc, pc);
-    double* o = y + n * YS + 2 * Ts + 8 * tv;
-#pragma unroll
-    for (int m = 0; m < 4; ++m) { o[m] = pc[m].r; o[4 + m] = pc[m].i; }
-  }
-  for (int e = threadIdx.x; e < N * Ts; e += BLOCK) {
-    const int n = e / Ts, t = e - n * Ts;
-    const double* x = sv + n * C * 10;
-    cx<double> acc = {0, 0};
-#pragma unroll 4
-    for (int c = 0; c < C; ++c) cfma(acc, cx<double>{w0l[t * C + c], w0l[Ts * C + t * C + c]}, cx<double>{x[c * 10], x[c * 10 + 1]});
-    y[n * YS + 2 * t] = acc.r;
-    y[n * YS + 2 * t + 1] = acc.i;
-  }
-  __syncthreads();
-  STAMP(2);
-  const int l8 = threadIdx.x & 7;
-  constexpr int NONE = 0x7fffffff;
-  for (int it = threadIdx.x >> 3; it < 2 * TT; it += BLOCK / 8) {
-    const int z = it / TT, t = it - z * TT;
-    int imin = NONE, imax = NONE;
-    double smin = 0, smax = 0;
-#pragma unroll 4
-    for (int n = l8; n < N; n += 8) {
-      double lo, hi;
-      if (t < Ts) {
-        const double val = y[n * YS + 2 * t + z];
-        lo = val;
-        hi = val * val;
-      } else {
-        const double* o = y + n * YS + 2 * Ts + 8 * (t - Ts) + 4 * z;
-        lo = hi = o[0] * o[0] - ((o[1] * o[1] + o[2] * o[2]) + o[3] * o[3]);
-      }
-      if (imin == NONE || lo < smin) { smin = lo; imin = n; }
-      if (imax == NONE || hi > smax) { smax = hi; imax = n; }
-    }
-#pragma unroll
-    for (int off = 4; off; off >>= 1) {
-      const double om = __shfl_xor(smin, off, 8), oM = __shfl_xor(smax, off, 8);
-      const int oi = __shfl_xor(imin, off, 8), oI = __shfl_xor(imax, off, 8);
-      if (oi != NONE && (imin == NONE || om < smin || (om == smin && oi < imin))) { smin = om; imin = oi; }
-      if (oI != NONE && (imax == NONE || oM > smax || (oM == smax && oI < imax))) { smax = oM; imax = oI; }
-    }
-    imin = __shfl(imin, 0, 8);
-    imax = __shfl(imax, 0, 8);
-    if (l8 < 2) idx[(((size_t)b * 2 + z) * TT + t) * 2 + l8] = l8 ? imax : imin;
-    const int nc = t < Ts ? 1 : 4, y0 = t < Ts ? 2 * t + z : 2 * Ts + 8 * (t - Ts) + 4 * z;
-    double mean[4] = {0, 0, 0, 0};
-    if (need_mean) {
-      for (int n = l8; n < N; n += 8)
-#pragma unroll
-        for (int m = 0; m < 4; ++m)
-          if (m < nc) mean[m] += y[n * YS + y0 + m];
-#pragma unroll
-      for (int off = 4; off; off >>= 1)
-#pragma unroll
-        for (int m = 0; m < 4; ++m) mean[m] += __shfl_xor(mean[m], off, 8);
-#pragma unroll
-      for (int m = 0; m < 4; ++m) mean[m] /= (double)N;
-    }
-    for (int k = l8; k < P * nc; k += 8) {
-      const int pb = k / nc, m = k - pb * nc;
-      auto pick = [&](int op) -> double {
-        if (op == LGN_POOL_MIN) return y[imin * YS + y0 + m];
-        if (op == LGN_POOL_MAX) return y[imax * YS + y0 + m];
-        return m == 0 ? mean[0] : (m == 1 ? mean[1] : (m == 2 ? mean[2] : mean[3]));
-      };
-      double val;
-      if (pool_avg(pool)) {
-        val = pick(pool_op(pool, 0));
-        for (int i = 1; i < PN; ++i) val += pick(pool_op(pool, i));
-        val /= (double)PN;
-      } else {
-        val = pick(pool_op(pool, pb));
-      }
-      if (t < Ts) {
-        lat_s[((size_t)z * B + b) * P * Ts + pb * Ts + t] = val;
-      } else {
-        const int tv = t - Ts;
-        lat_v[(((size_t)z * B + b) * P * Tv + pb * Tv + tv) * 4 + m] = val;
-        if constexpr (TO_LDS) lat_l[(pb * Tv + tv) * 8 + 4 * z + m] = val;
-      }
-    }
-  }
-}
 template <bool TO_LDS>
 __device__ __forceinline__ void enc_latent_mix_fwd_body(int B, int N, int C, int Ts, int Tv, double* lat_s, double* lat_v, double* lds,
                                                         double* lat_l) {
@@ -549,74 +389,6 @@
   else enc_latent_bwd_body<false>(B, N, C, Ts, Tv, pool, g_lat_s, g_lat_v, nullptr, idx, g_s, g_v, part, lds, pre);
 }
 
-__host__ __device__ inline size_t dec_in_fwd_doubles(int N, int C, int Tin) {
-  return 2 * (size_t)N * Tin + (size_t)Tin * 8 + (size_t)N * 8 + 4 * (size_t)C;
-}
-struct DecInFwdStage {
-  StageRegs<4> wg;
-  StageRegs<1> a0, a1, lr, li;
-  const double *wg1, *w0, *w1, *l0, *l1;
-  int N, C, Tin;
-  bool with_lat;
-  __device__ __forceinline__ void issue(int B, int N_, int C_, int Tin_, const double* __restrict__ lat_v, const double* __restrict__ wg1_,
-                                        const double* __restrict__ w0_, const double* __restrict__ w1_, bool with_lat_) {
-    N = N_; C = C_; Tin = Tin_; wg1 = wg1_; w0 = w0_; w1 = w1_; with_lat = with_lat_;
-    wg.issue(wg1, 2 * N * Tin);
-    a0.issue(w0, 2 * C); a1.issue(w1, 2 * C);
-    if (with_lat) {
-      l0 = lat_v + (size_t)blockIdx.x * Tin * 4; l1 = lat_v + ((size_t)B + blockIdx.x) * Tin * 4;
-      lr.issue(l0, Tin * 4); li.issue(l1, Tin * 4);
-    }
-  }
-  __device__ __forceinline__ void commit(double* lds) const {
-    double* wgl = lds;
-    double* latl = wgl + 2 * N * Tin;
-    double* w01 = latl + Tin * 8 + N * 8;
-    wg.commit(wg1, 2 * N * Tin, [&](int e, double x) { wgl[e] = x; });
-    a0.commit(w0, 2 * C, [&](int e, double x) { w01[e] = x; });
-    a1.commit(w1, 2 * C, [&](int e, double x) { w01[2 * C + e] = x; });
-    if (with_lat) {
-      lr.commit(l0, Tin * 4, [&](int e, double x) { latl[(e >> 2) * 8 + (e & 3)] = x; });
-      li.commit(l1, Tin * 4, [&](int e, double x) { latl[(e >> 2) * 8 + 4 + (e & 3)] = x; });
-    }
-  }
-};
-__device__ __forceinline__ void dec_input_fwd_body(int B, int N, int C, int Tin, double* pdec, double* s0, double* v0, double* lds) {
-  const double* wgl = lds;
-  const double* latl = wgl + 2 * N * Tin;
-  double* cartl = const_cast<double*>(latl) + Tin * 8;
-  const double* w01 = cartl + N * 8;
-  const int b = blockIdx.x;
-  const size_t plp = (size_t)B * N * 4, pl = (size_t)B * N * C;
-  STAMP(3);
-  for (int e = threadIdx.x; e < N * 4; e += BLOCK) {
-    const int n = e >> 2, m = e & 3;
-    cx<double> acc = {0, 0};
-#pragma unroll 8
-    for (int t = 0; t < Tin; ++t)
-      cfma(acc, cx<double>{wgl[n * Tin + t], wgl[N * Tin + n * Tin + t]}, cx<double>{latl[t * 8 + m], latl[t * 8 + 4 + m]});
-    cartl[n * 8 + m] = acc.r;
-    cartl[n * 8 + 4 + m] = acc.i;
-  }
-  __syncthreads();
-  STAMP(4);
-  for (int e = threadIdx.x; e < N * 4; e += BLOCK) {
-    const cx<double> pc = canon_cplx_m(cartl + (e >> 2) * 8, e & 3);
-    pdec[(size_t)b * N * 4 + e] = pc.r;
-    pdec[plp + (size_t)b * N * 4 + e] = pc.i;
-  }
-  for (int e = threadIdx.x; e < N * C; e += BLOCK) {
-    const int c = e % C;
-    s0[(size_t)b * N * C + e] = w01[c] - w01[C + c];
-    s0[pl + (size_t)b * N * C + e] = w01[C + c] + w01[c];
-  }
-  for (int e = threadIdx.x; e < N * C * 4; e += BLOCK) {
-    const int i = e >> 2, m = e & 3, n = i / C, c = i - n * C;
-    const cx<double> r = cmul(cx<double>{w01[2 * C + c], w01[3 * C + c]}, canon_cplx_m(cartl + n * 8, m));
-    v0[(size_t)b * N * C * 4 + e] = r.r;
-    v0[pl * 4 + (size_t)b * N * C * 4 + e] = r.i;
-  }
-}
 __global__ __launch_bounds__(BLOCK) void dec_input_fwd_kernel(int B, int N, int C, int Tin, const double* __restrict__ lat_v,
                                                              const double* __restrict__ wg1, const double* __restrict__ w0,
                                                              const double* __restrict__ w1, double* pdec, double* s0, double* v0) {
diff --git a/lgn-autoencoder_amd/csrc/ops.hpp b/lgn-autoencoder_amd/csrc/ops.hpp
--- a/lgn-autoencoder_amd/csrc/ops.hpp
+++ b/lgn-autoencoder_amd/csrc/ops.hpp
@@ -48,6 +48,7 @@
 bool level_bwd_carries_input(int N, int flags);
 bool level_dec_rebuilds(int N, int flags);
 bool level_fwd_carries_loss(int N, int flags);
+bool level_fwd_carries_junction(int N, int C, int CO, int CL, int Ts, int Tv, int pool, int flags);
 
 constexpr int MLP_MAX_LIN = 8;
 template <typename T>
diff --git a/lgn-autoencoder_amd/csrc/step.hip b/lgn-autoencoder_amd/csrc/step.hip
--- a/lgn-autoencoder_amd/csrc/step.hip
+++ b/lgn-autoencoder_amd/csrc/step.hip
@@ -301,9 +301,21 @@
   double jscale;
   double *recon, *loss_part, *g_v, *wpart;
 };
+struct JunctionStage {
+  const double *wl0, *wl1, *s, *v, *wg1, *w0, *w1;
+  double *lat_s, *lat_v;
+  int* idx;
+  double* pdec;
+  int CL, Ts, Tv, pool;
+};
+inline bool junction_rides(const lgn_net_desc& d) {
+  if (step_is_split(d) || d.enc_tables[0] || d.dec_tables[0]) return false;
+  return level_fwd_carries_junction(d.N, d.dec_channels[0], d.dec_channels[1], d.enc_channels[d.n_levels], d.tau_s, d.tau_v, d.latent_pool,
+                                    d.flags);
+}
 
 int levels_fwd(const lgn_net_desc& d, bool dec, const double* P, const int64_t* off, NetBuf& n, const double* pos, const uint8_t* mask,
-               hipStream_t st, const InputStage* in0, const LossStage* loss, bool eval, bool last_scalars) {
+               hipStream_t st, const InputStage* in0, const LossStage* loss, bool eval, bool last_scalars, const JunctionStage* jn = nullptr) {
   const Slots S{d.n_levels, d.mlp_nlin};
   const int* ch = dec ? d.dec_channels : d.enc_channels;
   for (int l = 0; l < d.n_levels; ++l) {
@@ -315,6 +327,11 @@
     if (l == 0 && !dec && in0) {
       a.in_w0 = in0->w0; a.in_w1 = in0->w1; a.in_s = n.s[0]; a.in_v = n.v[0];
       a.z1 = in0->z1; a.z1n = in0->z1n; a.z2 = in0->z2; a.z2n = in0->z2n;
+    }
+    if (l == 0 && dec && jn) {
+      a.jn_wl0 = jn->wl0; a.jn_wl1 = jn->wl1; a.jn_s = jn->s; a.jn_v = jn->v; a.jn_wg1 = jn->wg1; a.jn_w0 = jn->w0; a.jn_w1 = jn->w1;
+      a.jn_lat_s = jn->lat_s; a.jn_lat_v = jn->lat_v; a.jn_idx = jn->idx; a.jn_pdec = jn->pdec; a.jn_s0 = n.s[0]; a.jn_v0 = n.v[0];
+      a.jn_CL = jn->CL; a.jn_Ts = jn->Ts; a.jn_Tv = jn->Tv; a.jn_pool = pool_canon(jn->pool);
     }
     if (l + 1 == d.n_levels && dec && loss) {
       a.loss_wo1 = loss->wo1; a.loss_target = loss->target; a.loss_scale = loss->scale; a.loss_real = loss->method;
@@ -443,10 +460,11 @@
 }
 
 int decoder_fwd(const lgn_net_desc& d, const double* P, const int64_t* off, const double* lat_v, NetBuf& n, double* pdec, hipStream_t st,
-                bool with_input = true, const LossStage* loss = nullptr, bool eval = false, bool last_scalars = true) {
+                bool with_input = true, const LossStage* loss = nullptr, bool eval = false, bool last_scalars = true,
+                const JunctionStage* jn = nullptr) {
   if (with_input)
     LGN_TRY(dec_input_fwd(d.B, d.N, d.dec_channels[0], dec_tin(d), lat_v, P + off[1], P + off[2], P + off[3], pdec, n.s[0], n.v[0], st));
-  return levels_fwd(d, true, P, off, n, pdec, nullptr, st, nullptr, loss, eval, last_scalars);
+  return levels_fwd(d, true, P, off, n, pdec, nullptr, st, nullptr, loss, eval, last_scalars, jn);
 }
 
 int decoder_bwd(const lgn_net_desc& d, const double* P, double* G, const int64_t* off, const double* lat_v, const NetBuf& n,
@@ -939,11 +957,15 @@
   const bool split = step_is_split(d);
   LGN_TRY(encoder_fwd(d, params, enc_off, p4, mask, in_scalars, w.enc, w.lat_s, w.lat_v, w.idx, st, split ? nullptr : &ride,
                       split, eval, keep_s));
-  if (!split)
-    LGN_TRY(junction_fwd(d.B, d.N, d.enc_channels[L], d.tau_s, d.tau_v, d.latent_pool, keep_s ? w.enc.s[L] : nullptr, w.enc.v[L],
-                         params + enc_off[S.out0(false)], params + enc_off[S.out0(false) + 1], w.lat_s, w.lat_v, w.idx, d.dec_channels[0],
-                         params + dec_off[1], params + dec_off[2], params + dec_off[3], w.pdec, w.dec.s[0], w.dec.v[0], st));
-  return decoder_fwd(dd, params, dec_off, w.lat_v, w.dec, w.pdec, st, split, loss, eval, false);
+  const bool ride_jn = junction_rides(d);
+  const JunctionStage jn{params + enc_off[S.out0(false)], params + enc_off[S.out0(false) + 1], keep_s ? w.enc.s[L] : nullptr, w.enc.v[L],
+                         params + dec_off[1], params + dec_off[2], params + dec_off[3], w.lat_s, w.lat_v, w.idx, w.pdec,
+                         d.enc_channels[L], d.tau_s, d.tau_v, d.latent_pool};
+  if (!split && !ride_jn)
+    LGN_TRY(junction_fwd(d.B, d.N, jn.CL, jn.Ts, jn.Tv, jn.pool, jn.s, jn.v, jn.wl0, jn.wl1, jn.lat_s, jn.lat_v, jn.idx, d.dec_channels[0],
+                         jn.wg1, jn.w0, jn.w1, jn.pdec, w.dec.s[0], w.dec.v[0], st));
+  return decoder_fwd(dd, params, dec_off, w.lat_v, w.dec, w.pdec, st, split, loss, eval, false,
+                     ride_jn ? &jn : nullptr);
 }
 
 struct GenStep {
@@ -1336,6 +1358,7 @@
 long long lgn_junction_lds_bytes(int N, int CL, int Ts, int Tv, int pool, int C0) {
   return pool_valid(pool) ? (long long)junction_lds_bytes(N, CL, Ts, Tv, pool, C0) : -1;
 }
+int lgn_junction_rides(const lgn_net_desc* d) { return !check_desc(d) && !check_latent_match(*d) && junction_rides(*d) ? 1 : 0; }
 
 long long lgn_step_workspace_doubles(const lgn_net_desc* d) {
   if (check_desc(d) || check_latent_match(*d)) return -1;
diff --git a/lgn-autoencoder_amd/lgn/_native.py b/lgn-autoencoder_amd/lgn/_native.py
--- a/lgn-autoencoder_amd/lgn/_native.py
+++ b/lgn-autoencoder_amd/lgn/_native.py
@@ -109,7 +109,7 @@
 _NET_FLAG_ENV = {"LGN_AMD_NO_STATIC": 1, "LGN_AMD_DEC_PAIRWISE": 2, "LGN_AMD_LEVEL_V2": 4, "LGN_AMD_MLP_V1": 8,
                  "LGN_AMD_MOMENTS_V1": 16, "LGN_AMD_BWD_ORDERED": 64, "LGN_AMD_LIVE_SCALARS": 4096, "LGN_AMD_SPLIT_TAIL": 128, "LGN_AMD_DEC_UNFUSED": 256, "LGN_AMD_MOMENTS_SPLIT": 512,
                  "LGN_AMD_MLP_BWD1": 1024, "LGN_AMD_MLP_FULLTILE": 2048,
-                 "LGN_AMD_DEC_STORE_AG": 16384}
+                 "LGN_AMD_DEC_STORE_AG": 16384, "LGN_AMD_JUNCTION_LAUNCH": 32768}
 ACTIVATIONS = {"leakyrelu": 0, "relu": 1, "elu": 2, "sigmoid": 3, "logsigmoid": 4, "atan": 5}
 
 
@@ -150,6 +150,7 @@
     "lgn_local_bwd_static_f64": [_i] * 4 + [_vp] * 3 + [_ip] + [_vp] * 8,
     "lgn_local_bwd_f64": [_i] * 5 + [_tp] + [_vp] * 8,
     "lgn_step_param_slots": [_dp, _i],
+    "lgn_junction_rides": [_dp],
     "lgn_step_fwd_bwd_f64": [_dp, _vp, _vp, _ll, _vp, _vp, _vp, _vp, _vp, _vp, _vp, _ll, _vp, _vp, _lp, _vp, _vp, _vp],
     "lgn_encoder_fwd_f64": [_dp, _vp, _vp, _vp, _vp, _vp, _vp, _ll, _vp, _vp, _vp],
     "lgn_encoder_bwd_f64": [_dp, _vp, _vp, _ll, _vp, _vp, _vp, _vp, _vp, _ll, _vp, _vp, _vp, _ll, _vp],
```

New measurement: 1.138 million, median of 6. About the same (+0.5%).
